# anthonyhu/tumblr-emotions

Measured on AMD Instinct MI355X. Metric: training samples/sec (224x224 img + 32-tok text, batch 256), higher is better.
Workload: dtype f32; 1 GPU; joint train step (fwd+bwd+all-reduce+Adam): Inception-v1 224x224x3 + 300-d embedding + LSTM-512, T=32, V=10000, 15 classes, batch 256 per GPU, reference freeze (<=Mixed_5b conv weights frozen, all BN betas trainable), dropout 0.8, BN train mode; global_batch=256, per_gpu_batch=256, parallelism=dp1, launch=eager

## Files before the change

### include/ds_kernels.h

```cpp
#ifndef DS_KERNELS_H
#define DS_KERNELS_H

#include <stddef.h>
#include <stdint.h>

#ifdef __cplusplus
extern "C" {
#endif

#define DS_OK 0
#define DS_ERR_ARG (-1)
#define DS_ERR_LAUNCH (-2)
#define DS_ERR_WORKSPACE (-3)

#define DS_DTYPE_F32 0
#define DS_DTYPE_BF16 1

#define DS_EPI_BIAS 1
#define DS_EPI_RELU 2
#define DS_EPI_ACCUM 4
#define DS_EPI_STATS 8
#define DS_EPI_MASK 16
#define DS_EPI_BNSUMS 32

int ds_version(void);
const char *ds_last_error(void);

typedef struct ds_conv_desc {
    int32_t N, H, W;
    int32_t Cin;
    int32_t ldx;
    int32_t KH, KW, stride;
    int32_t pad_t, pad_l;
    int32_t OH, OW;
    int32_t Cout;
    int32_t ldz;
    int64_t w_tap_stride;
    int32_t w_n_stride;
    int32_t w_k_stride;
    int32_t flip;
    int32_t fold_cin;
    int32_t flags;
    int32_t ldmask;
    int32_t splits;
    int64_t z_split_stride;
    int32_t tile_nt;
    int32_t grid_x;
    int32_t dtype;
    int32_t x_dtype;
    int32_t partials;
    const float *norm_rstd;
    const float *norm_shift;
    const float *mask_rstd;
    const float *mask_shift;
    const struct ds_bn_bwd_on_load *bnb;
    int32_t mask_dtype;
    int32_t z_dtype;
    uint8_t *pool_argmax;
    const struct ds_bn_finalize_in_launch *fin;
} ds_conv_desc;

typedef struct ds_bn_finalize_in_launch {
    const float *beta;
    float *mean, *rstd, *shift;
    float *moving_mean, *moving_var;
    uint32_t *ticket;
    int64_t count;
    float eps, decay;
} ds_bn_finalize_in_launch;

typedef struct ds_bn_bwd_on_load {
    const float *mean, *rstd, *shift;
    const float *coef;
    int32_t nseg;
    int32_t c_end[3];
    int32_t ld[3];
    const float *dy[3];
} ds_bn_bwd_on_load;

#ifdef DS_TUNING
int ds_debug_conv_set_tile(int mt, int nt);
int ds_debug_conv_set_path(int path);
int ds_debug_conv_set_wide(int mode);
int ds_debug_conv_wino_allow_ablation(int on);
int ds_debug_conv_wino4_set_nb(int nb);
int ds_debug_conv_bf16_set_max_nb(int nb);
#endif
int ds_conv_igemm_partials(const ds_conv_desc *d);
int ds_conv_igemm_bnsums_supported(const ds_conv_desc *d);
int ds_conv_igemm_norm_supported(const ds_conv_desc *d);
int ds_conv_igemm_bnb_supported(const ds_conv_desc *d);
int ds_conv_igemm_pool3_supported(const ds_conv_desc *d);
int ds_conv_igemm_finalize_tickets(const ds_conv_desc *d);
int ds_conv_igemm(const ds_conv_desc *d, const float *x, const float *w, float *z, const float *bias,
                  const float *mask, float *stats, const float *pivot, void *stream);

size_t ds_weights_bf16_bytes(int32_t Cin, int32_t Cout, int32_t taps, int32_t dgrad);
int ds_weights_to_bf16(const float *w, void *wb, int32_t Cin, int32_t Cout, int32_t taps, int32_t dgrad, void *stream);
int ds_conv_bf16_supported(const ds_conv_desc *d);
int ds_conv_bf16_partials(const ds_conv_desc *d);
int ds_conv_bf16(const ds_conv_desc *d, const void *x, const void *wb, float *z, const void *mask, float *stats,
                 const float *pivot, void *stream);

size_t ds_weights_f32x3_bytes(int32_t Cin, int32_t Cout, int32_t taps, int32_t dgrad);
int ds_weights_to_f32x3(const float *w, void *wb, int32_t Cin, int32_t Cout, int32_t taps, int32_t dgrad, void *stream);
int ds_conv_f32x3_supported(const ds_conv_desc *d);
int ds_conv_f32x3_partials(const ds_conv_desc *d);
int ds_conv_f32x3(const ds_conv_desc *d, const float *x, const void *wb, float *z, const float *mask, float *stats,
                  const float *pivot, void *stream);

#define DS_FP8_E4M3 0
#define DS_FP8_E5M2 1
#define DS_AMAX_FLOATS 512
int ds_absmax(const void *x, int64_t n, int32_t x_dtype, float *amax, void *stream);
size_t ds_weights_fp8_bytes(int32_t Cin, int32_t Cout, int32_t taps, int32_t dgrad);
int ds_weights_to_fp8(const float *w, void *wq, float *wscale, int32_t Cin, int32_t Cout, int32_t taps, int32_t dgrad,
                      void *stream);
int ds_conv_fp8_supported(const ds_conv_desc *d);
int ds_conv_fp8_partials(const ds_conv_desc *d);
int ds_conv_fp8(const ds_conv_desc *d, const void *x, const float *x_amax, int32_t a_format, const void *wq,
                const float *wscale, float *z, const void *mask, float *stats, const float *pivot, void *stream);

int ds_conv_stem_partials(int32_t N, int32_t OH, int32_t OW);
int ds_conv_stem(const float *x, const float *w, float *z, float *stats, const float *pivot, int32_t N, int32_t H,
                 int32_t W, int32_t cin_store, int32_t Cout, int32_t ldz, void *stream);
int ds_conv_stem_pool_supported(int32_t H, int32_t W);
int ds_conv_stem_pool_partials(int32_t N, int32_t OH, int32_t OW);
int ds_conv_stem_pool(const float *x, const float *w, float *zmax, float *stats, const float *pivot, int32_t N, int32_t H,
                      int32_t W, int32_t cin_store, int32_t Cout, int32_t ldz, void *stream);
int ds_conv_stem_pool_bf16(const float *x, const float *w, float *zmax, float *stats, const float *pivot, int32_t N, int32_t H,
                           int32_t W, int32_t cin_store, int32_t Cout, int32_t ldz, void *stream);
int ds_conv_stem_dgrad_supported(int32_t H, int32_t W);
int ds_conv_stem_dgrad(const float *dz, const float *w, float *dx, int32_t N, int32_t H, int32_t W, int32_t cin_store,
                       int32_t ldx, void *stream);
int ds_conv_stem_bf16_partials(int32_t N, int32_t OH, int32_t OW);
int ds_conv_stem_bf16(const float *x, const float *w, float *z, float *stats, const float *pivot, int32_t N, int32_t H, int32_t W,
                      int32_t cin_store, int32_t Cout, int32_t ldz, void *stream);

int ds_wino_transform_weights(const float *w, float *u, int32_t Cin, int32_t Cout, int32_t dgrad, void *stream);
int ds_conv_wino_partials(int32_t N, int32_t H, int32_t W);
int ds_conv_wino(const float *x, const float *u, float *z, float *stats, const float *pivot, const float *ymask,
                 int32_t N, int32_t H, int32_t W, int32_t Cin, int32_t ldx, int32_t Cout, int32_t ldz, int32_t flags,
                 void *stream);

int ds_conv_wino4_supported(int32_t H, int32_t W, int32_t Cin, int32_t Cout);
int ds_conv_wino4_prefer(int32_t N, int32_t H, int32_t W, int32_t Cin, int32_t Cout);
int ds_wino4_transform_weights(const float *w, float *u, int32_t Cin, int32_t Cout, int32_t dgrad, void *stream);
int ds_conv_wino4_partials(int32_t N, int32_t H, int32_t W);
int ds_conv_wino4(const float *x, const float *u, float *z, float *stats, const float *pivot, const float *ymask,
                  int32_t N, int32_t H, int32_t W, int32_t Cin, int32_t ldx, int32_t Cout, int32_t ldz, int32_t flags,
                  void *stream);
int ds_conv_wino4_splitk_choose(int32_t N, int32_t H, int32_t W, int32_t Cin, int32_t Cout);
int ds_conv_wino4_splitk_partials(int32_t N, int32_t H, int32_t W);
size_t ds_conv_wino4_splitk_workspace(int32_t N, int32_t H, int32_t W, int32_t Cout, int32_t splits);
int ds_conv_wino4_splitk(const float *x, const float *u, float *z, float *stats, const float *pivot, const float *ymask,
                         int32_t y_dtype, int32_t N, int32_t H, int32_t W, int32_t Cin, int32_t ldx, int32_t Cout, int32_t ldz,
                         int32_t flags, int32_t splits, void *ws, size_t ws_bytes, void *stream);
int ds_wino4_transform_weights_bf16x2(const float *w, void *u2, int32_t Cin, int32_t Cout, int32_t dgrad, void *stream);
int ds_conv_wino4_bf16x2(const float *x, const void *u2, float *z, float *stats, const float *pivot, const void *ymask,
                         int32_t y_dtype , int32_t N,
                         int32_t H, int32_t W, int32_t Cin, int32_t ldx, int32_t Cout, int32_t ldz, int32_t flags, void *stream);
int ds_conv_wino4_bf16x2_x16(const void *x16, const void *u2, float *z, float *stats, const float *pivot, const void *ymask,
                             int32_t y_dtype, int32_t N, int32_t H, int32_t W, int32_t Cin, int32_t ldx, int32_t Cout, int32_t ldz,
                             int32_t flags, void *stream);

#define DS_CONV_FWD 0
#define DS_CONV_DGRAD 1
#define DS_ARITH_F32 0
#define DS_ARITH_BF16 1
#define DS_ARITH_FP8 2
#define DS_ARITH_F32X3 3
#define DS_FAM_IGEMM 0
#define DS_FAM_WINO2 1
#define DS_FAM_WINO4 2
#define DS_FAM_STEM 3
#define DS_FAM_BF16D 4
#define DS_FAM_FP8D 5
#define DS_FAM_F32X3 6
#define DS_FAM_WINO4H 7
#define DS_FAM_STEM_POOL 8
#define DS_FAM_STEM_DGRAD 9
#define DS_PLAN_NO_WINO 1u
#define DS_PLAN_NO_WINO4 2u
#define DS_PLAN_NO_STEM_DIRECT 4u
#define DS_PLAN_NO_BF16_DIRECT 8u
#define DS_PLAN_ACT16 16u
#define DS_PLAN_FP8_EVERYWHERE 64u
#define DS_PLAN_FP8_WIDE_RULE 128u
#define DS_PLAN_NO_WINO4H 256u
#define DS_PLAN_STEM_POOL 512u
#define DS_PLAN_NO_SPLITK 1024u
#define DS_PLAN_PACKED_RGB 32u
typedef struct ds_conv_layer_plan {
    ds_conv_desc d;
    int32_t family;
    int32_t role, arith;
    int32_t partials;
    int32_t w_cin, w_cout, k;
    int32_t a_format;
    int32_t x16_ok;
    int64_t w_bytes;
    int64_t wscale_floats;
    double alg_flops;
    int32_t splitk;
    int32_t reserved0;
    int64_t ws_bytes;
} ds_conv_layer_plan;
typedef struct ds_conv_io {
    const float *bias;
    const float *mask;
    float *stats;
    const float *pivot;
    const float *x_amax;
    const float *wscale;
    const ds_bn_finalize_in_launch *fin;
    void *ws;
    size_t ws_bytes;
} ds_conv_io;
int ds_conv_plan(ds_conv_layer_plan *plan, int32_t role, int32_t arith, uint32_t options, int32_t N, int32_t H, int32_t W,
                 int32_t w_cin, int32_t w_cout, int32_t k, int32_t stride, int32_t ldx, int32_t ldz, int32_t flags);
int ds_conv_plan_set_flags(ds_conv_layer_plan *plan, int32_t flags);
int ds_conv_plan_enable_bnsums(ds_conv_layer_plan *plan, int32_t ldy);
int ds_conv_plan_norm_supported(const ds_conv_layer_plan *plan);
int ds_conv_plan_bnb_supported(const ds_conv_layer_plan *plan);
int ds_conv_plan_enable_pool3(ds_conv_layer_plan *plan, uint8_t *argmax);
int ds_conv_plan_finalize_tickets(const ds_conv_layer_plan *plan);
int ds_conv_prepare_weights(const ds_conv_layer_plan *plan, const float *w_hwio, void *w_prepared, float *wscale,
                            void *stream);
int ds_conv_run(const ds_conv_layer_plan *plan, const void *x, const void *w, float *z, const ds_conv_io *io, void *stream);

size_t ds_conv_wgrad_workspace(const ds_conv_desc *d);
int ds_conv_wgrad(const ds_conv_desc *d, const float *x, const float *dz, int32_t lddz, float *dw,
                  void *ws, size_t ws_bytes, void *stream);

int ds_bn_finalize(const float *stats, int32_t P, int64_t count, int32_t C, const float *beta, const float *pivot,
                   float eps, float decay, float *mean, float *rstd, float *shift, float *moving_mean,
                   float *moving_var, void *stream);

int ds_bn_finalize_centered(const float *stats, int32_t P, int64_t count, int32_t C, const float *beta, const float *pivot,
                            float eps, float decay, float *mean, float *rstd, float *shift, float *moving_mean,
                            float *moving_var, float *mean_c, float *shift_c, void *stream);
typedef struct ds_bn_finalize_job {
    const float *stats;
    int32_t P, C;
    int64_t count;
    const float *beta;
    const float *pivot;
    float *mean, *rstd, *shift;
    float *moving_mean, *moving_var;
} ds_bn_finalize_job;
int ds_bn_finalize_multi(const ds_bn_finalize_job *jobs, int32_t njobs, float eps, float decay, void *stream);

int ds_bn_finalize_apply_relu(const float *stats, int32_t P, int64_t count, int32_t C, const float *beta, const float *pivot,
                              float eps, float decay, float *mean, float *rstd, float *shift, float *moving_mean,
                              float *moving_var, const float *z, int64_t M, const struct ds_segments *dst, uint32_t *ticket,
                              void *stream);

typedef struct ds_segments {
    int32_t nseg;
    int32_t c_begin[4];
    int32_t c_end[4];
    int32_t ld[4];
    void *ptr[4];
    int32_t dtype[4];
    float *amax[4];
    const float *ptr2[4];
} ds_segments;
int ds_bn_apply_relu(const float *z, int64_t M, int32_t C, const float *rstd, const float *shift,
                     const ds_segments *dst, void *stream);
int ds_bn_apply_relu_z16(const void *z16, int64_t M, int32_t C, const float *rstd, const float *shift,
                         const ds_segments *dst, void *stream);
int ds_bn_infer_prepare(const float *beta, const float *moving_mean, const float *moving_var, float eps,
                        int32_t C, float *rstd, float *shift, void *stream);

int ds_bn_bwd_partials(int64_t M, int32_t C);
int ds_bn_bwd_reduce(const void *z, int32_t ldz, int32_t z_dtype, const ds_segments *dy, int64_t M, int32_t C,
                     const float *mean, const float *rstd, const float *shift, float *partials, void *stream);
int ds_bn_bwd_finalize(const float *partials, int32_t P, int64_t M, int32_t C, float *dbeta, float *coef,
                       void *stream);
typedef struct ds_bn_sum_segments {
    int32_t nseg;
    int32_t c_begin[4], c_end[4];
    int32_t P[4];
    int32_t kind[4];
    const float *s[4];
    const float *q[4];
    int32_t P2[4];
    const float *s2[4];
    const float *q2[4];
} ds_bn_sum_segments;
int ds_bn_bwd_finalize_segs(const ds_bn_sum_segments *sg, int64_t M, int32_t C, const float *beta, float *dbeta,
                            float *coef, void *stream);
int ds_bn_bwd_finalize_multi(const ds_bn_sum_segments *sg, int64_t M, int32_t C, const float *const *beta,
                             float *const *dbeta, float *coef, void *stream);
int ds_bn_bwd_finalize_apply(const ds_bn_sum_segments *sg, const float *beta, float *dbeta, const float *const *beta_v,
                             float *const *dbeta_v, float *coef, const float *z, int32_t ldz, const ds_segments *dy, int64_t M,
                             int32_t C, const float *mean, const float *rstd, const float *shift, void *dz, int32_t dz_dtype,
                             int32_t lddz, float *amax, uint32_t *ticket, void *stream);
int ds_bn_bwd_apply(const float *z, int32_t ldz, const ds_segments *dy, int64_t M, int32_t C, const float *mean,
                    const float *rstd, const float *shift, const float *coef, float *dz, float *amax, void *stream);
int ds_bn_bwd_apply_bf16(const float *z, int32_t ldz, const ds_segments *dy, int64_t M, int32_t C, const float *mean,
                         const float *rstd, const float *shift, const float *coef, void *dz16, int32_t lddz, float *amax,
                         void *stream);

int ds_bn_bwd_apply_z16(const void *z16, int32_t ldz, const ds_segments *dy, int64_t M, int32_t C, const float *mean,
                        const float *rstd, const float *shift, const float *coef, void *dz16, int32_t lddz, float *amax,
                        void *stream);

int ds_maxpool_fwd(const void *x, void *y, uint8_t *argmax, int32_t N, int32_t H, int32_t W, int32_t C,
                   int32_t k, int32_t stride, int32_t pad_t, int32_t pad_l, int32_t OH, int32_t OW,
                   int32_t act_dtype, void *stream);
int ds_maxpool_bn_relu_fwd(const float *z, const float *rstd, const float *shift, void *y, uint8_t *argmax,
                           int32_t N, int32_t H, int32_t W, int32_t C, int32_t k, int32_t stride, int32_t pad_t,
                           int32_t pad_l, int32_t OH, int32_t OW, int32_t y_dtype, float *amax, void *stream);
int ds_bn_pool_bwd_partials(int32_t N, int32_t OH, int32_t OW, int32_t C);
int ds_bn_pool_bwd_reduce(const float *z, const float *dpool, const uint8_t *argmax, int32_t N, int32_t H, int32_t W,
                          int32_t C, int32_t pad_t, int32_t pad_l, int32_t OH, int32_t OW, const float *mean,
                          const float *rstd, const float *shift, float *partials, void *stream);
int ds_bn_pool_bwd_apply(const float *z, const float *dpool, const uint8_t *argmax, int32_t N, int32_t H, int32_t W,
                         int32_t C, int32_t pad_t, int32_t pad_l, int32_t OH, int32_t OW, const float *mean,
                         const float *rstd, const float *shift, const float *coef, float *dz, void *stream);
int ds_maxpool_bwd(const float *dy, const uint8_t *argmax, float *dx, int32_t accumulate, int32_t N,
                   int32_t H, int32_t W, int32_t C, int32_t k, int32_t stride, int32_t pad_t, int32_t pad_l,
                   int32_t OH, int32_t OW, void *stream);

int ds_maxpool3_bwd_sums_partials(int32_t N, int32_t W, int32_t C);
int ds_maxpool3_bwd_sums(const float *dy, const uint8_t *argmax, float *dx, int32_t accumulate, const void *y,
                         int32_t y_dtype, int32_t N, int32_t H, int32_t W, int32_t C, float *partials, void *stream);

int ds_maxpool3_bwd_dy16(const void *dy16, const uint8_t *argmax, float *dx, int32_t accumulate, const void *y, int32_t y_dtype,
                         int32_t N, int32_t H, int32_t W, int32_t C, float *partials, void *stream);

int ds_avgpool_dropout_fwd(const float *x, int32_t N, int32_t HW, int32_t C, float keep, uint64_t seed,
                           const uint64_t *seed_dev, const float *mask_in, float *mask_out, float *out,
                           void *stream);
int ds_avgpool_dropout_bwd(const float *dout, const float *mask, int32_t N, int32_t HW, int32_t C,
                           float keep, float *dx, void *stream);

int ds_gather_rows(const float *table, const int64_t *ids, float *out, int32_t B, int32_t T, int32_t D,
                   int64_t table_rows, int32_t time_major, void *stream);

int ds_embedding_grad(const float *dx, const int64_t *ids, float *dtable, int32_t B, int32_t T, int32_t D,
                      int64_t table_rows, int32_t time_major, void *stream);

int ds_lstm_cell_fwd(float *gates, const float *rec_slabs, int32_t nslabs, int64_t slab_stride,
                     const float *c_prev, const float *h_prev, const int64_t *seq_len, int32_t t, int32_t B,
                     int32_t H, float forget_bias, float *c_out, float *h_out, void *stream);
int ds_lstm_cell_bwd(const float *acts, const float *c_t, const float *c_prev, const float *dh,
                     const float *dh_slabs, int32_t nslabs, int64_t slab_stride, const float *dc,
                     const int64_t *seq_len, int32_t t, int32_t B, int32_t H, float *dgates, float *dc_prev,
                     float *dh_carry, void *stream);

int ds_seq_sort_desc(const int64_t *seq_len, int32_t B, int32_t T, int32_t *perm, int64_t *len_sorted, void *stream);
int ds_permute_rows(const void *src, int64_t lds, void *dst, int64_t ldd, const int32_t *perm, int32_t rows, int32_t cols,
                    int32_t elem_bytes, int32_t gather, void *stream);
#define DS_LSTM_SKIP_MASKED 256
int ds_lstm_seq_supported(int32_t B, int32_t H);
size_t ds_lstm_seq_workspace(int32_t B, int32_t H);
int ds_lstm_seq_fwd(float *gates, const float *wh, int32_t ldw, float *h, float *c, const int64_t *seq_len, int32_t T,
                    int32_t B, int32_t H, float forget_bias, int32_t rows, void *ws, size_t ws_bytes, void *stream);
int ds_lstm_seq_bwd(const float *acts, const float *wh, int32_t ldw, const float *c, const float *dh_last,
                    int32_t ld_dh, const int64_t *seq_len, int32_t T, int32_t B, int32_t H, float *dgates, int32_t rows,
                    void *ws, size_t ws_bytes, void *stream);
int ds_lstm_seq_status(void *ws, int32_t B);
#ifdef DS_TUNING
int ds_debug_lstm_seq_set_profile(void *buf);
int ds_debug_lstm_seq_set_profile_bwd(void *buf);
#endif

int ds_softmax_ce(const float *logits, const int64_t *labels, int32_t B, int32_t C, float grad_scale,
                  const float *grad_scale_dev, float *loss, float *dlogits, void *stream);

int ds_adam_tf(float *theta, const float *g, float *m, float *v, int64_t n, int64_t n_wd, float wd,
               float grad_scale, float lr_t, const float *lr_t_dev, float beta1, float beta2, float eps,
               void *stream);

int ds_sumsq(const float *x, int64_t n, float *scratch, float *out, void *stream);
int ds_colsum(const float *x, int64_t M, int32_t C, int32_t ld, float *scratch, float *out, void *stream);
int ds_slab_epilogue(const float *slabs, int32_t splits, int64_t slab_stride, int32_t lds, int64_t M, int32_t N, float *out,
                     int32_t ldo, const float *bias, const float *mask, int32_t ldmask, int32_t flags, void *stream);
int ds_copy2d(const float *src, int32_t lds, float *dst, int32_t ldd, int64_t rows, int32_t cols,
              void *stream);
int ds_pad_channels(const float *src, int32_t cs, float *dst, int32_t cd, int64_t pixels, void *stream);
int ds_fill(float *dst, int64_t n, float value, void *stream);

#ifdef __cplusplus
}
#endif
#endif
```

### tumblr_emotions_amd/_lib.py

```python
import ctypes as C
import os

_HERE = os.path.dirname(os.path.abspath(__file__))
LIB_PATH = os.environ.get("DS_LIB") or os.path.join(_HERE, "libds_kernels.so")

def tuning_env(name, default=None):
    return os.environ.get(name, default) if os.environ.get("DS_LIB") else default


DS_EPI_BIAS, DS_EPI_RELU, DS_EPI_ACCUM, DS_EPI_STATS, DS_EPI_MASK, DS_EPI_BNSUMS = 1, 2, 4, 8, 16, 32
DS_DTYPE_F32, DS_DTYPE_BF16 = 0, 1
DS_FP8_E4M3, DS_FP8_E5M2 = 0, 1
DS_CONV_FWD, DS_CONV_DGRAD = 0, 1
DS_LSTM_SKIP_MASKED = 256
DS_ARITH_F32, DS_ARITH_BF16, DS_ARITH_FP8, DS_ARITH_F32X3 = 0, 1, 2, 3
DS_FAM_IGEMM, DS_FAM_WINO2, DS_FAM_WINO4, DS_FAM_STEM, DS_FAM_BF16D, DS_FAM_FP8D, DS_FAM_F32X3, DS_FAM_WINO4H, DS_FAM_STEM_POOL = range(9)
DS_FAM_STEM_DGRAD = 9
DS_PLAN_NO_WINO, DS_PLAN_NO_WINO4, DS_PLAN_NO_STEM_DIRECT, DS_PLAN_NO_BF16_DIRECT, DS_PLAN_ACT16, DS_PLAN_PACKED_RGB = 1, 2, 4, 8, 16, 32
DS_PLAN_FP8_EVERYWHERE, DS_PLAN_FP8_WIDE_RULE, DS_PLAN_NO_WINO4H, DS_PLAN_STEM_POOL = 64, 128, 256, 512
DS_PLAN_NO_SPLITK = 1024


class ConvDesc(C.Structure):
    _fields_ = [
        ("N", C.c_int32), ("H", C.c_int32), ("W", C.c_int32), ("Cin", C.c_int32), ("ldx", C.c_int32),
        ("KH", C.c_int32), ("KW", C.c_int32), ("stride", C.c_int32), ("pad_t", C.c_int32), ("pad_l", C.c_int32),
        ("OH", C.c_int32), ("OW", C.c_int32), ("Cout", C.c_int32), ("ldz", C.c_int32),
        ("w_tap_stride", C.c_int64), ("w_n_stride", C.c_int32), ("w_k_stride", C.c_int32),
        ("flip", C.c_int32), ("fold_cin", C.c_int32), ("flags", C.c_int32), ("ldmask", C.c_int32),
        ("splits", C.c_int32), ("z_split_stride", C.c_int64),
        ("tile_nt", C.c_int32), ("grid_x", C.c_int32), ("dtype", C.c_int32), ("x_dtype", C.c_int32),
        ("partials", C.c_int32),
        ("norm_rstd", C.c_void_p), ("norm_shift", C.c_void_p), ("mask_rstd", C.c_void_p), ("mask_shift", C.c_void_p),
        ("bnb", C.c_void_p), ("mask_dtype", C.c_int32), ("z_dtype", C.c_int32), ("pool_argmax", C.c_void_p), ("fin", C.c_void_p),
    ]


class BnBwdOnLoad(C.Structure):
    _fields_ = [("mean", C.c_void_p), ("rstd", C.c_void_p), ("shift", C.c_void_p), ("coef", C.c_void_p),
                ("nseg", C.c_int32), ("c_end", C.c_int32 * 3), ("ld", C.c_int32 * 3), ("dy", C.c_void_p * 3)]


class BnFinalizeInLaunch(C.Structure):
    _fields_ = [("beta", C.c_void_p), ("mean", C.c_void_p), ("rstd", C.c_void_p), ("shift", C.c_void_p),
                ("moving_mean", C.c_void_p), ("moving_var", C.c_void_p), ("ticket", C.c_void_p), ("count", C.c_int64),
                ("eps", C.c_float), ("decay", C.c_float)]


class LayerPlanStruct(C.Structure):
    _fields_ = [("d", ConvDesc), ("family", C.c_int32), ("role", C.c_int32), ("arith", C.c_int32), ("partials", C.c_int32),
                ("w_cin", C.c_int32), ("w_cout", C.c_int32), ("k", C.c_int32), ("a_format", C.c_int32), ("x16_ok", C.c_int32),
                ("w_bytes", C.c_int64), ("wscale_floats", C.c_int64), ("alg_flops", C.c_double), ("splitk", C.c_int32),
                ("reserved0", C.c_int32), ("ws_bytes", C.c_int64)]


class ConvIO(C.Structure):
    _fields_ = [("bias", C.c_void_p), ("mask", C.c_void_p), ("stats", C.c_void_p), ("pivot", C.c_void_p),
                ("x_amax", C.c_void_p), ("wscale", C.c_void_p), ("fin", C.c_void_p), ("ws", C.c_void_p), ("ws_bytes", C.c_size_t)]


class Segments(C.Structure):
    _fields_ = [("nseg", C.c_int32), ("c_begin", C.c_int32 * 4), ("c_end", C.c_int32 * 4),
                ("ld", C.c_int32 * 4), ("ptr", C.c_void_p * 4), ("dtype", C.c_int32 * 4),
                ("amax", C.c_void_p * 4), ("ptr2", C.c_void_p * 4)]


class BnFinalizeJob(C.Structure):
    _fields_ = [("stats", C.c_void_p), ("P", C.c_int32), ("C", C.c_int32), ("count", C.c_int64), ("beta", C.c_void_p),
                ("pivot", C.c_void_p), ("mean", C.c_void_p), ("rstd", C.c_void_p), ("shift", C.c_void_p),
                ("moving_mean", C.c_void_p), ("moving_var", C.c_void_p)]


class SumSegments(C.Structure):
    _fields_ = [("nseg", C.c_int32), ("c_begin", C.c_int32 * 4), ("c_end", C.c_int32 * 4), ("P", C.c_int32 * 4),
                ("kind", C.c_int32 * 4), ("s", C.c_void_p * 4), ("q", C.c_void_p * 4), ("P2", C.c_int32 * 4),
                ("s2", C.c_void_p * 4), ("q2", C.c_void_p * 4)]


_P = C.c_void_p
_i32, _i64, _f32, _u64 = C.c_int32, C.c_int64, C.c_float, C.c_uint64
_CD = C.POINTER(ConvDesc)
_SG = C.POINTER(Segments)
_SS = C.POINTER(SumSegments)
_LP = C.POINTER(LayerPlanStruct)
_IO = C.POINTER(ConvIO)

SIGNATURES = {
    "ds_version": (C.c_int, []),
    "ds_last_error": (C.c_char_p, []),
    "ds_conv_igemm_partials": (C.c_int, [_CD]),
    "ds_conv_igemm_bnsums_supported": (C.c_int, [_CD]),
    "ds_conv_igemm_norm_supported": (C.c_int, [_CD]),
    "ds_conv_igemm_bnb_supported": (C.c_int, [_CD]),
    "ds_conv_igemm_pool3_supported": (C.c_int, [_CD]),
    "ds_conv_igemm_finalize_tickets": (C.c_int, [_CD]),
    "ds_conv_igemm": (C.c_int, [_CD, _P, _P, _P, _P, _P, _P, _P, _P]),
    "ds_weights_bf16_bytes": (C.c_size_t, [_i32, _i32, _i32, _i32]),
    "ds_weights_to_bf16": (C.c_int, [_P, _P, _i32, _i32, _i32, _i32, _P]),
    "ds_conv_bf16_supported": (C.c_int, [_CD]),
    "ds_conv_bf16_partials": (C.c_int, [_CD]),
    "ds_conv_bf16": (C.c_int, [_CD, _P, _P, _P, _P, _P, _P, _P]),
    "ds_weights_f32x3_bytes": (C.c_size_t, [_i32, _i32, _i32, _i32]),
    "ds_weights_to_f32x3": (C.c_int, [_P, _P, _i32, _i32, _i32, _i32, _P]),
    "ds_conv_f32x3_supported": (C.c_int, [_CD]),
    "ds_conv_f32x3_partials": (C.c_int, [_CD]),
    "ds_conv_f32x3": (C.c_int, [_CD, _P, _P, _P, _P, _P, _P, _P]),
    "ds_absmax": (C.c_int, [_P, _i64, _i32, _P, _P]),
    "ds_weights_fp8_bytes": (C.c_size_t, [_i32, _i32, _i32, _i32]),
    "ds_weights_to_fp8": (C.c_int, [_P, _P, _P, _i32, _i32, _i32, _i32, _P]),
    "ds_conv_fp8_supported": (C.c_int, [_CD]),
    "ds_conv_fp8_partials": (C.c_int, [_CD]),
    "ds_conv_fp8": (C.c_int, [_CD, _P, _P, _i32, _P, _P, _P, _P, _P, _P, _P]),
    "ds_conv_stem_partials": (C.c_int, [_i32, _i32, _i32]),
    "ds_conv_stem_bf16_partials": (C.c_int, [_i32, _i32, _i32]),
    "ds_conv_stem": (C.c_int, [_P, _P, _P, _P, _P, _i32, _i32, _i32, _i32, _i32, _i32, _P]),
    "ds_conv_stem_bf16": (C.c_int, [_P, _P, _P, _P, _P, _i32, _i32, _i32, _i32, _i32, _i32, _P]),
    "ds_conv_stem_pool_supported": (C.c_int, [_i32, _i32]),
    "ds_conv_stem_pool_partials": (C.c_int, [_i32, _i32, _i32]),
    "ds_conv_stem_pool": (C.c_int, [_P, _P, _P, _P, _P, _i32, _i32, _i32, _i32, _i32, _i32, _P]),
    "ds_conv_stem_pool_bf16": (C.c_int, [_P, _P, _P, _P, _P, _i32, _i32, _i32, _i32, _i32, _i32, _P]),
    "ds_conv_stem_dgrad_supported": (C.c_int, [_i32, _i32]),
    "ds_conv_stem_dgrad": (C.c_int, [_P, _P, _P, _i32, _i32, _i32, _i32, _i32, _P]),
    "ds_wino_transform_weights": (C.c_int, [_P, _P, _i32, _i32, _i32, _P]),
    "ds_conv_wino_partials": (C.c_int, [_i32, _i32, _i32]),
    "ds_conv_wino": (C.c_int, [_P, _P, _P, _P, _P, _P, _i32, _i32, _i32, _i32, _i32, _i32, _i32, _i32, _P]),
    "ds_conv_wino4_supported": (C.c_int, [_i32, _i32, _i32, _i32]),
    "ds_conv_wino4_prefer": (C.c_int, [_i32, _i32, _i32, _i32, _i32]),
    "ds_wino4_transform_weights": (C.c_int, [_P, _P, _i32, _i32, _i32, _P]),
    "ds_conv_wino4_partials": (C.c_int, [_i32, _i32, _i32]),
    "ds_conv_wino4_splitk_choose": (C.c_int, [_i32, _i32, _i32, _i32, _i32]),
    "ds_conv_wino4_splitk_partials": (C.c_int, [_i32, _i32, _i32]),
    "ds_conv_wino4_splitk_workspace": (C.c_size_t, [_i32, _i32, _i32, _i32, _i32]),
    "ds_conv_wino4_splitk": (C.c_int, [_P, _P, _P, _P, _P, _P, _i32, _i32, _i32, _i32, _i32, _i32, _i32, _i32, _i32, _i32, _P, C.c_size_t, _P]),
    "ds_conv_wino4": (C.c_int, [_P, _P, _P, _P, _P, _P, _i32, _i32, _i32, _i32, _i32, _i32, _i32, _i32, _P]),
    "ds_conv_wino4_bf16x2": (C.c_int, [_P, _P, _P, _P, _P, _P, _i32, _i32, _i32, _i32, _i32, _i32, _i32, _i32, _i32, _P]),
    "ds_conv_wino4_bf16x2_x16": (C.c_int, [_P, _P, _P, _P, _P, _P, _i32, _i32, _i32, _i32, _i32, _i32, _i32, _i32, _i32, _P]),
    "ds_wino4_transform_weights_bf16x2": (C.c_int, [_P, _P, _i32, _i32, _i32, _P]),
    "ds_conv_plan": (C.c_int, [_LP, _i32, _i32, C.c_uint32] + [_i32] * 10),
    "ds_conv_plan_set_flags": (C.c_int, [_LP, _i32]),
    "ds_conv_plan_enable_bnsums": (C.c_int, [_LP, _i32]),
    "ds_conv_plan_norm_supported": (C.c_int, [_LP]),
    "ds_conv_plan_bnb_supported": (C.c_int, [_LP]),
    "ds_conv_plan_enable_pool3": (C.c_int, [_LP, C.c_void_p]),
    "ds_conv_plan_finalize_tickets": (C.c_int, [_LP]),
    "ds_conv_prepare_weights": (C.c_int, [_LP, _P, _P, _P, _P]),
    "ds_conv_run": (C.c_int, [_LP, _P, _P, _P, _IO, _P]),
    "ds_conv_wgrad_workspace": (C.c_size_t, [_CD]),
    "ds_conv_wgrad": (C.c_int, [_CD, _P, _P, _i32, _P, _P, C.c_size_t, _P]),
    "ds_bn_finalize": (C.c_int, [_P, _i32, _i64, _i32, _P, _P, _f32, _f32, _P, _P, _P, _P, _P, _P]),
    "ds_bn_finalize_centered": (C.c_int, [_P, _i32, _i64, _i32, _P, _P, _f32, _f32, _P, _P, _P, _P, _P, _P, _P, _P]),
    "ds_bn_apply_relu": (C.c_int, [_P, _i64, _i32, _P, _P, _SG, _P]),
    "ds_bn_apply_relu_z16": (C.c_int, [_P, _i64, _i32, _P, _P, _SG, _P]),
    "ds_bn_bwd_apply_z16": (C.c_int, [_P, _i32, _SG, _i64, _i32, _P, _P, _P, _P, _P, _i32, _P, _P]),
    "ds_bn_infer_prepare": (C.c_int, [_P, _P, _P, _f32, _i32, _P, _P, _P]),
    "ds_bn_bwd_partials": (C.c_int, [_i64, _i32]),
    "ds_bn_bwd_reduce": (C.c_int, [_P, _i32, _i32, _SG, _i64, _i32, _P, _P, _P, _P, _P]),
    "ds_bn_bwd_finalize_segs": (C.c_int, [_SS, _i64, _i32, _P, _P, _P, _P]),
    "ds_bn_bwd_finalize": (C.c_int, [_P, _i32, _i64, _i32, _P, _P, _P]),
    "ds_bn_bwd_finalize_multi": (C.c_int, [_SS, _i64, _i32, _P, _P, _P, _P]),
    "ds_bn_finalize_multi": (C.c_int, [_P, _i32, _f32, _f32, _P]),
    "ds_bn_finalize_apply_relu": (C.c_int, [_P, _i32, _i64, _i32, _P, _P, _f32, _f32, _P, _P, _P, _P, _P, _P, _i64, _SG, _P, _P]),
    "ds_bn_bwd_finalize_apply": (C.c_int, [_SS, _P, _P, _P, _P, _P, _P, _i32, _SG, _i64, _i32, _P, _P, _P, _P, _i32, _i32, _P, _P, _P]),
    "ds_bn_bwd_apply": (C.c_int, [_P, _i32, _SG, _i64, _i32, _P, _P, _P, _P, _P, _P, _P]),
    "ds_bn_bwd_apply_bf16": (C.c_int, [_P, _i32, _SG, _i64, _i32, _P, _P, _P, _P, _P, _i32, _P, _P]),
    "ds_maxpool_fwd": (C.c_int, [_P, _P, _P] + [_i32] * 11 + [_P]),
    "ds_maxpool_bn_relu_fwd": (C.c_int, [_P, _P, _P, _P, _P] + [_i32] * 11 + [_P, _P]),
    "ds_bn_pool_bwd_partials": (C.c_int, [_i32, _i32, _i32, _i32]),
    "ds_bn_pool_bwd_reduce": (C.c_int, [_P, _P, _P] + [_i32] * 8 + [_P, _P, _P, _P, _P]),
    "ds_bn_pool_bwd_apply": (C.c_int, [_P, _P, _P] + [_i32] * 8 + [_P, _P, _P, _P, _P, _P]),
    "ds_maxpool_bwd": (C.c_int, [_P, _P, _P] + [_i32] * 11 + [_P]),
    "ds_maxpool3_bwd_sums_partials": (C.c_int, [_i32, _i32, _i32]),
    "ds_maxpool3_bwd_sums": (C.c_int, [_P, _P, _P, _i32, _P, _i32, _i32, _i32, _i32, _i32, _P, _P]),
    "ds_maxpool3_bwd_dy16": (C.c_int, [_P, _P, _P, _i32, _P, _i32, _i32, _i32, _i32, _i32, _P, _P]),
    "ds_avgpool_dropout_fwd": (C.c_int, [_P, _i32, _i32, _i32, _f32, _u64, _P, _P, _P, _P, _P]),
    "ds_avgpool_dropout_bwd": (C.c_int, [_P, _P, _i32, _i32, _i32, _f32, _P, _P]),
    "ds_gather_rows": (C.c_int, [_P, _P, _P, _i32, _i32, _i32, _i64, _i32, _P]),
    "ds_embedding_grad": (C.c_int, [_P, _P, _P, _i32, _i32, _i32, _i64, _i32, _P]),
    "ds_lstm_cell_fwd": (C.c_int, [_P, _P, _i32, _i64, _P, _P, _P, _i32, _i32, _i32, _f32, _P, _P, _P]),
    "ds_lstm_cell_bwd": (C.c_int, [_P, _P, _P, _P, _P, _i32, _i64, _P, _P, _i32, _i32, _i32, _P, _P, _P, _P]),
    "ds_seq_sort_desc": (C.c_int, [_P, _i32, _i32, _P, _P, _P]),
    "ds_permute_rows": (C.c_int, [_P, _i64, _P, _i64, _P, _i32, _i32, _i32, _i32, _P]),
    "ds_lstm_seq_supported": (C.c_int, [_i32, _i32]),
    "ds_lstm_seq_workspace": (C.c_size_t, [_i32, _i32]),
    "ds_lstm_seq_fwd": (C.c_int, [_P, _P, _i32, _P, _P, _P, _i32, _i32, _i32, _f32, _i32, _P, C.c_size_t, _P]),
    "ds_lstm_seq_bwd": (C.c_int, [_P, _P, _i32, _P, _P, _i32, _P, _i32, _i32, _i32, _P, _i32, _P, C.c_size_t, _P]),
    "ds_lstm_seq_status": (C.c_int, [_P, _i32]),
    "ds_softmax_ce": (C.c_int, [_P, _P, _i32, _i32, _f32, _P, _P, _P, _P]),
    "ds_adam_tf": (C.c_int, [_P, _P, _P, _P, _i64, _i64, _f32, _f32, _f32, _P, _f32, _f32, _f32, _P]),
    "ds_sumsq": (C.c_int, [_P, _i64, _P, _P, _P]),
    "ds_colsum": (C.c_int, [_P, _i64, _i32, _i32, _P, _P, _P]),
    "ds_slab_epilogue": (C.c_int, [_P, _i32, _i64, _i32, _i64, _i32, _P, _i32, _P, _P, _i32, _i32, _P]),
    "ds_copy2d": (C.c_int, [_P, _i32, _P, _i32, _i64, _i32, _P]),
    "ds_pad_channels": (C.c_int, [_P, _i32, _P, _i32, _i64, _P]),
    "ds_fill": (C.c_int, [_P, _i64, _f32, _P]),
}

_lib = None


DEBUG_SIGNATURES = {
    "ds_debug_conv_set_tile": (C.c_int, [C.c_int, C.c_int]),
    "ds_debug_conv_set_path": (C.c_int, [C.c_int]),
    "ds_debug_conv_set_wide": (C.c_int, [C.c_int]),
    "ds_debug_conv_wino_allow_ablation": (C.c_int, [C.c_int]),
    "ds_debug_conv_wino4_set_nb": (C.c_int, [C.c_int]),
    "ds_debug_conv_bf16_set_max_nb": (C.c_int, [C.c_int]),
    "ds_debug_lstm_seq_set_profile": (C.c_int, [_P]),
    "ds_debug_lstm_seq_set_profile_bwd": (C.c_int, [_P]),
}
TUNING_LIB_PATH = os.path.join(_HERE, "libds_kernels_tuning.so")
_tuning = None


def _bind(lib, table):
    for name, (res, args) in table.items():
        fn = getattr(lib, name)
        fn.restype = res
        fn.argtypes = args


def load_tuning():
    global _tuning
    if _tuning is None:
        if not os.path.exists(TUNING_LIB_PATH):
            raise RuntimeError("tumblr_emotions_amd: %s not found -- `make -C tumblr_emotions_amd/csrc` builds it" % TUNING_LIB_PATH)
        lib = C.CDLL(TUNING_LIB_PATH)
        _bind(lib, SIGNATURES)
        _bind(lib, DEBUG_SIGNATURES)
        _tuning = lib
    return _tuning


class tuning_library:

    def __enter__(self):
        global _lib
        self._saved = load()
        _lib = load_tuning()
        return _lib

    def __exit__(self, *exc):
        global _lib
        _lib = self._saved
        return False


def load():
    global _lib
    if _lib is not None:
        return _lib
    if not os.path.exists(LIB_PATH):
        raise RuntimeError(
            "tumblr_emotions_amd: %s not found -- build it with `python -c 'import __graft_entry__ as g; "
            "g.build()'` or `make -C tumblr_emotions_amd/csrc`.  There is no CPU fallback." % LIB_PATH)
    if os.environ.get("DS_LIB"):
        import sys
        sys.stderr.write("tumblr_emotions_amd: DS_LIB overrides the kernel library: %s\n" % LIB_PATH)
    lib = C.CDLL(LIB_PATH)
    _bind(lib, SIGNATURES)
    if hasattr(lib, "ds_debug_conv_set_tile"):
        _bind(lib, DEBUG_SIGNATURES)
    _lib = lib
    return lib


def check(rc, what):
    if rc != 0:
        raise RuntimeError("%s failed (%d): %s" % (what, rc, load().ds_last_error().decode()))
```

### tumblr_emotions_amd/csrc/conv_wgrad.hip

```cpp
#include <stdio.h>
#include <stdlib.h>
#include "ds_common.h"

typedef float f32x16 __attribute__((ext_vector_type(16)));
typedef float f32x4 __attribute__((ext_vector_type(4)));
typedef unsigned int u32x4 __attribute__((ext_vector_type(4)));

namespace {

constexpr int TJ = 128;
constexpr int TP = 16;

struct WgradParams {
    ds_conv_desc d;
    const float *x;
    const float *dz;
    float *out;
    int lddz;
    int M;
    int ci_tiles;
    int pix_per_split;
    int x_vec, z_vec;
    unsigned x_bytes, z_bytes;
    float inv_ohw, inv_ow;
    int slabs;
};

constexpr unsigned kOOB = 0x80000000u;

__device__ __forceinline__ __amdgpu_buffer_rsrc_t make_srd(const void *p, unsigned bytes) {
    return __builtin_amdgcn_make_buffer_rsrc(const_cast<void *>(p), 0, (int)bytes, 0x00020000);
}

__device__ __forceinline__ f32x4 load4(__amdgpu_buffer_rsrc_t r, unsigned off, bool ok, bool vec, int valid) {
    if (vec) return __builtin_bit_cast(f32x4, __builtin_amdgcn_raw_buffer_load_b128(r, ok ? off : kOOB, 0, 0));
    f32x4 v;
#pragma unroll
    for (int j = 0; j < 4; ++j)
        v[j] = __builtin_bit_cast(float, __builtin_amdgcn_raw_buffer_load_b32(r, (ok && j < valid) ? off + 4 * j : kOOB, 0, 0));
    return v;
}

__device__ __forceinline__ int fdiv(int a, int b, float inv) {
    int q = (int)((float)a * inv);
    int r = a - q * b;
    if (r < 0) --q;
    if (r >= b) ++q;
    return q;
}

template <int TIT>
__global__ __launch_bounds__(256) void conv_wgrad_kernel(const WgradParams p) {
    constexpr int LDX = TIT + 4, LDZ = TJ + 4;
    constexpr int WNW = TIT == 128 ? 2 : 4;
    constexpr int CW = TJ / WNW;
    constexpr int BS = CW / 32;
    constexpr int XQ = TIT / 4;
    constexpr int XROWS = 256 / XQ;
    constexpr int XP = TP / XROWS;
    __shared__ __attribute__((aligned(16))) float smem[2 * TP * LDX + 2 * TP * LDZ];
    float *Xs = smem;
    float *Zs = smem + 2 * TP * LDX;
    const ds_conv_desc &d = p.d;
    const int tid = threadIdx.x, lane = tid & 63;
    const int wave = __builtin_amdgcn_readfirstlane(tid >> 6);
    const int wm = TIT == 128 ? wave >> 1 : 0, wn = TIT == 128 ? wave & 1 : wave;
    const int li = lane & 31, lk = lane >> 5;
    const int tap = blockIdx.x / p.ci_tiles;
    const int i0 = (blockIdx.x % p.ci_tiles) * TIT;
    const int j0 = blockIdx.y * TJ;
    const int split = blockIdx.z;
    const int dh = tap / d.KW, dw = tap % d.KW;
    const int ohw = d.OH * d.OW;
    const int m_begin = split * p.pix_per_split;
    int m_end = m_begin + p.pix_per_split;
    if (m_end > p.M) m_end = p.M;

    int it_valid = (d.Cin - (i0 + wm * 64) + 31) / 32;
    it_valid = it_valid < 0 ? 0 : (it_valid > 2 ? 2 : it_valid);
    int jt_valid = (d.Cout - (j0 + wn * CW) + 31) / 32;
    jt_valid = jt_valid < 0 ? 0 : (jt_valid > BS ? BS : jt_valid);

    f32x16 acc[2][BS];
#pragma unroll
    for (int a = 0; a < 2; ++a)
#pragma unroll
        for (int b = 0; b < BS; ++b)
#pragma unroll
            for (int r = 0; r < 16; ++r) acc[a][b][r] = 0.f;

    const int xrow = tid / XQ, xc4 = (tid % XQ) * 4;
    const int zrow = tid >> 5, zc4 = (tid & 31) * 4;
    f32x4 rx[XP], rz[2];
    const __amdgpu_buffer_rsrc_t srd_x = make_srd(p.x, p.x_bytes);
    const __amdgpu_buffer_rsrc_t srd_z = make_srd(p.dz, p.z_bytes);
    const int cx = i0 + xc4, cz = j0 + zc4;
    const bool small = p.M < (1 << 24);

    auto load_tile = [&](int mt0) {
#pragma unroll
        for (int i = 0; i < XP; ++i) {
            const int m = mt0 + xrow + XROWS * i;
            const bool rv = m < m_end;
            const int mm = rv ? m : 0;
            const int n = small ? fdiv(mm, ohw, p.inv_ohw) : mm / ohw;
            const int r = mm - n * ohw;
            const int oh = small ? fdiv(r, d.OW, p.inv_ow) : r / d.OW;
            const int ow = r - oh * d.OW;
            const int ih = oh * d.stride - d.pad_t + dh, iw = ow * d.stride - d.pad_l + dw;
            const int iwc = d.fold_cin > 0 ? iw + cx / d.fold_cin : iw;
            const bool okx = rv && (unsigned)ih < (unsigned)d.H && (unsigned)iwc < (unsigned)d.W && cx < d.Cin;
            const unsigned offx = (unsigned)(((n * d.H + ih) * d.W + iw) * d.ldx + cx);
            rx[i] = load4(srd_x, offx * 4u, okx, p.x_vec, d.Cin - cx);
        }
#pragma unroll
        for (int i = 0; i < 2; ++i) {
            const int m = mt0 + zrow + 8 * i;
            const bool okz = m < m_end && cz < d.Cout;
            const unsigned offz = (unsigned)(m < m_end ? m : 0) * (unsigned)p.lddz + (unsigned)cz;
            rz[i] = load4(srd_z, offz * 4u, okz, p.z_vec, d.Cout - cz);
        }
    };
    auto store_tile = [&](int buf) {
#pragma unroll
        for (int i = 0; i < XP; ++i)
            *reinterpret_cast<f32x4 *>(Xs + (buf * TP + xrow + XROWS * i) * LDX + xc4) = rx[i];
#pragma unroll
        for (int i = 0; i < 2; ++i)
            *reinterpret_cast<f32x4 *>(Zs + (buf * TP + zrow + 8 * i) * LDZ + zc4) = rz[i];
    };
    auto compute = [&](int buf) {
        const float *xs = Xs + buf * TP * LDX + wm * 64 + li;
        const float *zs = Zs + buf * TP * LDZ + wn * CW + li;
#pragma unroll
        for (int s = 0; s < TP / 2; ++s) {
            const int row = 2 * s + lk;
            float af[2], bf[BS];
            af[0] = xs[row * LDX];
            af[1] = xs[row * LDX + 32];
#pragma unroll
            for (int b = 0; b < BS; ++b) bf[b] = zs[row * LDZ + 32 * b];
#pragma unroll
            for (int a = 0; a < 2; ++a)
#pragma unroll
                for (int b = 0; b < BS; ++b)
                    if (a < it_valid && b < jt_valid)
                        acc[a][b] = __builtin_amdgcn_mfma_f32_32x32x2f32(af[a], bf[b], acc[a][b], 0, 0, 0);
        }
    };

    const int KT = (m_end - m_begin + TP - 1) / TP;
    if (KT > 0) {
        load_tile(m_begin);
        store_tile(0);
        __syncthreads();
        for (int kt = 0; kt < KT; ++kt) {
            const int cur = kt & 1;
            if (kt + 1 < KT) load_tile(m_begin + (kt + 1) * TP);
            compute(cur);
            if (kt + 1 < KT) store_tile(cur ^ 1);
            __syncthreads();
        }
    }

    float *out = p.out + (int64_t)split * (d.KH * d.KW) * d.Cin * d.Cout + (int64_t)tap * d.Cin * d.Cout;
#pragma unroll
    for (int a = 0; a < 2; ++a)
#pragma unroll
        for (int b = 0; b < BS; ++b) {
            const int col = j0 + wn * CW + b * 32 + li;
#pragma unroll
            for (int r = 0; r < 16; ++r) {
                const int row = i0 + wm * 64 + a * 32 + (r & 3) + 8 * (r >> 2) + 4 * lk;
                if (row < d.Cin && col < d.Cout) out[(int64_t)row * d.Cout + col] = acc[a][b][r];
            }
        }
}


#ifndef DS_WG_U
#define DS_WG_U 4
#endif
template <int W>
__device__ __forceinline__ f32x4 loadw(__amdgpu_buffer_rsrc_t r, unsigned off) {
    f32x4 v = {0.f, 0.f, 0.f, 0.f};
    if constexpr (W == 4) {
        v = __builtin_bit_cast(f32x4, __builtin_amdgcn_raw_buffer_load_b128(r, off, 0, 0));
    } else if constexpr (W == 2) {
        typedef unsigned int u32x2 __attribute__((ext_vector_type(2)));
        typedef float f32x2 __attribute__((ext_vector_type(2)));
        const f32x2 t = __builtin_bit_cast(f32x2, __builtin_amdgcn_raw_buffer_load_b64(r, off, 0, 0));
        v[0] = t[0]; v[1] = t[1];
    } else {
        v[0] = __builtin_bit_cast(float, __builtin_amdgcn_raw_buffer_load_b32(r, off, 0, 0));
    }
    return v;
}

template <int AI, int BJ>
__global__ __launch_bounds__(256, (AI * BJ > 8) ? 1 : 2) void wgrad_direct_kernel(const WgradParams p) {
    constexpr int NACC = AI * BJ, U = DS_WG_U;
    __shared__ __attribute__((aligned(16))) float red[2 * NACC * 16 * 64];
    const ds_conv_desc &d = p.d;
    const int tid = threadIdx.x, lane = tid & 63;
    const int wave = __builtin_amdgcn_readfirstlane(tid >> 6);
    const int li = lane & 31, lk = lane >> 5;
    const int co_tiles = (d.Cout + 32 * BJ - 1) / (32 * BJ);
    const int split = (int)(blockIdx.x % (unsigned)p.slabs);
    int bid = (int)(blockIdx.x / (unsigned)p.slabs);
    const int jt = bid % co_tiles; bid /= co_tiles;
    const int itile = bid % p.ci_tiles;
    const int tap = bid / p.ci_tiles;
    const int dh = tap / d.KW, dw = tap % d.KW;
    const int ci0 = itile * 32 * AI, co0 = jt * 32 * BJ;
    const int ci = ci0 + AI * li, co = co0 + BJ * li;
    const bool ci_ok = ci < d.Cin, co_ok = co < d.Cout;
    const __amdgpu_buffer_rsrc_t srd_x = make_srd(p.x, p.x_bytes);
    const __amdgpu_buffer_rsrc_t srd_z = make_srd(p.dz, p.z_bytes);

    const int m_begin = split * p.pix_per_split;
    int m_end = m_begin + p.pix_per_split;
    if (m_end > p.M) m_end = p.M;
    int q = (m_end - m_begin + 3) / 4;
    q = (q + 1) & ~1;
    const int wb = m_begin + wave * q;
    int we = wb + q;
    if (we > m_end) we = m_end;
    const int steps = we > wb ? (we - wb + 1) / 2 : 0;

    int m = wb + lk;
    const int ohw = d.OH * d.OW;
    int oh = 0, ow = 0;
    unsigned offx, offz;
    {
        const int mm = m < p.M ? m : 0;
        const int n = mm / ohw;
        const int r = mm - n * ohw;
        oh = r / d.OW;
        ow = r - oh * d.OW;
        const int ih = oh * d.stride - d.pad_t + dh, iw = ow * d.stride - d.pad_l + dw;
        offx = ((unsigned)((n * d.H + ih) * d.W + iw) * (unsigned)d.ldx + (unsigned)ci) * 4u;
        offz = ((unsigned)mm * (unsigned)p.lddz + (unsigned)co) * 4u;
    }
    const unsigned ldx4 = (unsigned)d.ldx * 4u;
    const unsigned step_x = 2u * (unsigned)d.stride * ldx4;
    const unsigned row_x = (unsigned)((d.W - d.OW) * d.stride) * ldx4;
    const unsigned img_x = (unsigned)((d.H - d.OH * d.stride) * d.W) * ldx4;
    const unsigned step_z = 2u * (unsigned)p.lddz * 4u;
    auto lo_of = [](int pad, int tap, int stride) { const int v = pad - tap; return v <= 0 ? 0 : (v + stride - 1) / stride; };
    auto hi_of = [](int pad, int tap, int stride, int ext, int oext) {
        const int v = ext - 1 + pad - tap;
        const int h = v < 0 ? -1 : v / stride;
        return h > oext - 1 ? oext - 1 : h;
    };
    const int lo_h = lo_of(d.pad_t, dh, d.stride), lo_w = lo_of(d.pad_l, dw, d.stride);
    const unsigned span_h = (unsigned)(hi_of(d.pad_t, dh, d.stride, d.H, d.OH) - lo_h);
    const unsigned span_w = (unsigned)(hi_of(d.pad_l, dw, d.stride, d.W, d.OW) - lo_w);
    const int OWc = d.OW, OHc = d.OH;
    auto offsets = [&](unsigned &ox, unsigned &oz) {
        const bool mv = m < we;
        const bool in = (unsigned)(oh - lo_h) <= span_h && (unsigned)(ow - lo_w) <= span_w;
        oz = (mv && co_ok) ? offz : kOOB;
        ox = (mv && ci_ok && in) ? offx : kOOB;
        m += 2;
        offz += step_z;
        offx += step_x;
        ow += 2;
#pragma unroll
        for (int rep = 0; rep < 2; ++rep) {
            if (rep == 1 && OWc > 1) break;
            const bool wrap = ow >= OWc;
            ow = wrap ? ow - OWc : ow;
            oh += wrap ? 1 : 0;
            offx += wrap ? row_x : 0u;
            const bool wrap2 = oh >= OHc;
            oh = wrap2 ? oh - OHc : oh;
            offx += wrap2 ? img_x : 0u;
        }
    };

    f32x16 acc[AI][BJ];
#pragma unroll
    for (int a = 0; a < AI; ++a)
#pragma unroll
        for (int b = 0; b < BJ; ++b)
#pragma unroll
            for (int r = 0; r < 16; ++r) acc[a][b][r] = 0.f;

    f32x4 xa[U], zb[U];
#pragma unroll
    for (int u = 0; u < U; ++u) {
        unsigned ox, oz;
        offsets(ox, oz);
        xa[u] = loadw<AI>(srd_x, ox);
        zb[u] = loadw<BJ>(srd_z, oz);
    }
    for (int s = 0; s < steps; s += U) {
#pragma unroll
        for (int u = 0; u < U; ++u) {
            const f32x4 a4 = xa[u], b4 = zb[u];
            unsigned ox, oz;
            offsets(ox, oz);
            xa[u] = loadw<AI>(srd_x, ox);
            zb[u] = loadw<BJ>(srd_z, oz);
#pragma unroll
            for (int a = 0; a < AI; ++a)
#pragma unroll
                for (int b = 0; b < BJ; ++b)
                    acc[a][b] = __builtin_amdgcn_mfma_f32_32x32x2f32(a4[a], b4[b], acc[a][b], 0, 0, 0);
        }
    }

    auto put = [&](int slot) {
#pragma unroll
        for (int a = 0; a < AI; ++a)
#pragma unroll
            for (int b = 0; b < BJ; ++b)
#pragma unroll
                for (int r4 = 0; r4 < 4; ++r4) {
                    f32x4 v = {acc[a][b][4 * r4], acc[a][b][4 * r4 + 1], acc[a][b][4 * r4 + 2], acc[a][b][4 * r4 + 3]};
                    *reinterpret_cast<f32x4 *>(red + ((slot * NACC + a * BJ + b) * 4 + r4) * 256 + lane * 4) = v;
                }
    };
    auto get = [&](int slot) {
#pragma unroll
        for (int a = 0; a < AI; ++a)
#pragma unroll
            for (int b = 0; b < BJ; ++b)
#pragma unroll
                for (int r4 = 0; r4 < 4; ++r4) {
                    const f32x4 v = *reinterpret_cast<const f32x4 *>(red + ((slot * NACC + a * BJ + b) * 4 + r4) * 256 + lane * 4);
#pragma unroll
                    for (int e = 0; e < 4; ++e) acc[a][b][4 * r4 + e] += v[e];
                }
    };
    if (wave >= 2) put(wave - 2);
    __syncthreads();
    if (wave < 2) get(wave);
    __syncthreads();
    if (wave == 1) put(0);
    __syncthreads();
    if (wave != 0) return;
    get(0);

    float *out = p.out + (int64_t)split * (d.KH * d.KW) * d.Cin * d.Cout + (int64_t)tap * d.Cin * d.Cout;
    if (!co_ok) return;
#pragma unroll
    for (int a = 0; a < AI; ++a)
#pragma unroll
        for (int r = 0; r < 16; ++r) {
            const int row = ci0 + AI * ((r & 3) + 8 * (r >> 2) + 4 * lk) + a;
            if (row < d.Cin) {
                float *o = out + (int64_t)row * d.Cout + co;
                if constexpr (BJ == 4) {
                    *reinterpret_cast<f32x4 *>(o) = f32x4{acc[a][0][r], acc[a][1][r], acc[a][2][r], acc[a][3][r]};
                } else if constexpr (BJ == 2) {
                    typedef float f32x2 __attribute__((ext_vector_type(2)));
                    *reinterpret_cast<f32x2 *>(o) = f32x2{acc[a][0][r], acc[a][1][r]};
                } else {
                    *o = acc[a][0][r];
                }
            }
        }
}

__global__ __launch_bounds__(256) void splitk_reduce_kernel(const float *ws, float *dw, int64_t n, int splits) {
    for (int64_t i = (int64_t)blockIdx.x * 256 + threadIdx.x; i < n; i += (int64_t)gridDim.x * 256) {
        float s = 0.f;
        for (int k = 0; k < splits; ++k) s += ws[(int64_t)k * n + i];
        dw[i] = s;
    }
}

int pick_ti(const ds_conv_desc *d) {
    const int p128 = (d->Cin + 127) / 128 * 128, p64 = (d->Cin + 63) / 64 * 64;
    return (p128 - p64) * 5 >= p128 ? 64 : 128;
}

int pick_splits(const ds_conv_desc *d, int64_t M) {
    const int ti = pick_ti(d);
    const int tiles = d->KH * d->KW * ((d->Cin + ti - 1) / ti) * ((d->Cout + TJ - 1) / TJ);
    static int occ = 0, minpix = 0;
    if (!occ) {
        const char *e = ds::tune_env("DS_WGRAD_OCC");
        occ = e ? atoi(e) : 3;
        e = ds::tune_env("DS_WGRAD_MINPIX");
        minpix = e ? atoi(e) : 64;
    }
    int splits = (occ * ds::kCUs + tiles - 1) / tiles;
    const int max_splits = (int)((M + minpix - 1) / minpix);
    if (splits > max_splits) splits = max_splits;
    if (splits < 1) splits = 1;
    return splits;
}

struct WgradPlan {
    int direct;
    int ai, bj;
    int splits;
};

int max_width(int C, int ld, uintptr_t ptr) {
    for (int w = 4; w > 1; w >>= 1)
        if (C % w == 0 && ld % w == 0 && (ptr & (4 * w - 1)) == 0) return w;
    return 1;
}

bool direct_ok(const ds_conv_desc *d, int64_t M) {
    static int mode = -1;
    if (mode < 0) {
        const char *e = ds::tune_env("DS_WGRAD_DIRECT");
        mode = e ? atoi(e) : 1;
    }
    return mode && d->fold_cin == 0 && M >= 512;
}

WgradPlan plan_direct(const ds_conv_desc *d, int64_t M, int wx, int wz, int only_ai = 0, int only_bj = 0) {
    WgradPlan best = {};
    double best_cost = 1e30;
    static const int kSlabs[] = {1, 2, 4, 8, 16, 24, 32, 40, 48, 56, 64};
    const double wbytes = (double)d->KH * d->KW * d->Cin * d->Cout * 4.0;
    for (int ai = 1; ai <= wx; ai *= 2)
        for (int bj = 1; bj <= wz; bj *= 2) {
            if ((only_ai && ai != only_ai) || (only_bj && bj != only_bj)) continue;
            const int nacc = ai * bj;
            const int occ = nacc > 8 ? 1 : (nacc > 4 ? 2 : 3);
            const int tiles = d->KH * d->KW * ((d->Cin + 32 * ai - 1) / (32 * ai)) * ((d->Cout + 32 * bj - 1) / (32 * bj));
            for (int slabs : kSlabs) {
                if (slabs > 1 && M / slabs < 256) break;
                const int xcds = slabs >= 8 ? 8 : slabs;
                const double per_xcd = (double)tiles * slabs / 8.0;
                const double slots = 32.0 * occ;
                double rounds = (double)(int64_t)(per_xcd / slots);
                if (rounds * slots < per_xcd) rounds += 1.0;
                const double steps = (double)M / slabs / 8.0;
                const double step_cycles = nacc * 64.0 > 160.0 ? nacc * 64.0 : 160.0;
                const double t_wg = steps * step_cycles + 1500.0 + nacc * 350.0;
                const double t_red = slabs > 1 ? 6000.0 + slabs * wbytes / 1500.0 : 0.0;
                const double cost = rounds * t_wg + t_red;
                (void)xcds;
                if (cost < best_cost) {
                    best_cost = cost;
                    best.direct = 1; best.ai = ai; best.bj = bj; best.splits = slabs;
                }
            }
        }
    return best;
}

WgradPlan plan_wgrad(const ds_conv_desc *d, int64_t M, const float *x, const float *dz, int lddz, const float *dw,
                     const void *ws) {
    if (direct_ok(d, M)) {
        const uintptr_t zalign = (uintptr_t)dz | (uintptr_t)dw | (uintptr_t)ws;
        const int wx = max_width(d->Cin, d->ldx, (uintptr_t)x), wz = max_width(d->Cout, lddz, zalign);
        WgradPlan pl = plan_direct(d, M, wx, wz);
        if (const char *e = ds::tune_env("DS_WGRAD_FORCE")) {
            int a = 0, b = 0, sl = 0;
            if (sscanf(e, "%d,%d,%d", &a, &b, &sl) == 3) {
                if ((a && a <= wx) || (b && b <= wz)) {
                    const WgradPlan f = plan_direct(d, M, wx, wz, a <= wx ? a : 0, b <= wz ? b : 0);
                    if (f.direct) pl = f;
                }
                if (sl) pl.splits = sl;
            }
        }
        return pl;
    }
    WgradPlan pl = {};
    pl.splits = pick_splits(d, M);
    return pl;
}

}

extern "C" size_t ds_conv_wgrad_workspace(const ds_conv_desc *d) {
    const int64_t M = (int64_t)d->N * d->OH * d->OW;
    int splits = pick_splits(d, M);
    if (direct_ok(d, M)) {
        splits = 1;
        for (int wx = 1; wx <= 4; wx *= 2)
            for (int wz = 1; wz <= 4; wz *= 2) {
                const int sp = plan_direct(d, M, wx, wz).splits;
                splits = sp > splits ? sp : splits;
            }
    }
    if (splits == 1) return 0;
    return (size_t)splits * d->KH * d->KW * d->Cin * d->Cout * sizeof(float);
}

extern "C" int ds_conv_wgrad(const ds_conv_desc *d, const float *x, const float *dz, int32_t lddz, float *dw,
                             void *ws, size_t ws_bytes, void *stream) {
    DS_REQUIRE(d && x && dz && dw, "ds_conv_wgrad: null argument");
    const int64_t M = (int64_t)d->N * d->OH * d->OW;
    DS_REQUIRE(M < (1ll << 31), "ds_conv_wgrad: M too large");
    DS_REQUIRE(d->fold_cin == 0 || (d->KW == 1 && d->ldx == d->fold_cin && d->fold_cin % 4 == 0 && d->Cin % d->fold_cin == 0),
               "ds_conv_wgrad: fold_cin needs KW=1, ldx==fold_cin, fold_cin %% 4 == 0");
    const WgradPlan pl = plan_wgrad(d, M, x, dz, lddz, dw, ws);
    if (ds::tune_env("DS_WGRAD_DEBUG"))
        fprintf(stderr, "wgrad M=%lld Cin=%d Cout=%d k=%d: direct=%d ai=%d bj=%d slabs=%d\n", (long long)M, d->Cin, d->Cout, d->KH,
                pl.direct, pl.ai, pl.bj, pl.splits);
    const int splits = pl.splits;
    const size_t need = splits == 1 ? 0 : (size_t)splits * d->KH * d->KW * d->Cin * d->Cout * sizeof(float);
    if (need > 0 && (ws == nullptr || ws_bytes < need)) {
        ds::set_error("ds_conv_wgrad: workspace %zu bytes < required %zu", ws_bytes, need);
        return DS_ERR_WORKSPACE;
    }
    WgradParams p;
    p.d = *d;
    p.x = x; p.dz = dz; p.lddz = lddz;
    p.out = splits == 1 ? dw : (float *)ws;
    p.M = (int)M;
    const int64_t x_elems = ((int64_t)d->N * d->H * d->W - 1) * d->ldx + d->Cin;
    const int64_t z_elems = (M - 1) * lddz + d->Cout;
    DS_REQUIRE(x_elems * 4 < (1ll << 31) && z_elems * 4 < (1ll << 31), "ds_conv_wgrad: operand larger than 2 GiB (split the batch)");
    p.x_bytes = (unsigned)(x_elems * 4);
    p.z_bytes = (unsigned)(z_elems * 4);
    p.inv_ohw = 1.0f / (float)(d->OH * d->OW);
    p.inv_ow = 1.0f / (float)d->OW;
    p.x_vec = (d->ldx % 4 == 0) && (d->Cin % 4 == 0) && (((uintptr_t)x & 15) == 0);
    p.z_vec = (lddz % 4 == 0) && (d->Cout % 4 == 0) && (((uintptr_t)dz & 15) == 0);
    hipStream_t s = (hipStream_t)stream;
    int pps = (int)((M + splits - 1) / splits);
    if (pl.direct) {
        p.ci_tiles = (d->Cin + 32 * pl.ai - 1) / (32 * pl.ai);
        p.pix_per_split = (pps + 7) / 8 * 8;
        const int co_tiles = (d->Cout + 32 * pl.bj - 1) / (32 * pl.bj);
        p.slabs = splits;
        const dim3 grid((unsigned)(d->KH * d->KW * p.ci_tiles * co_tiles * splits));
#define DS_WG(A, B) if (pl.ai == A && pl.bj == B) hipLaunchKernelGGL((wgrad_direct_kernel<A, B>), grid, dim3(256), 0, s, p);
        DS_WG(4, 4) DS_WG(4, 2) DS_WG(4, 1) DS_WG(2, 4) DS_WG(2, 2) DS_WG(2, 1) DS_WG(1, 4) DS_WG(1, 2) DS_WG(1, 1)
#undef DS_WG
    } else {
        const int ti = pick_ti(d);
        p.ci_tiles = (d->Cin + ti - 1) / ti;
        p.pix_per_split = ((pps + TP - 1) / TP) * TP;
        dim3 grid(d->KH * d->KW * p.ci_tiles, (d->Cout + TJ - 1) / TJ, splits);
        if (ti == 64) hipLaunchKernelGGL(conv_wgrad_kernel<64>, grid, dim3(256), 0, s, p);
        else hipLaunchKernelGGL(conv_wgrad_kernel<128>, grid, dim3(256), 0, s, p);
    }
    if (splits > 1) {
        const int64_t n = (int64_t)d->KH * d->KW * d->Cin * d->Cout;
        hipLaunchKernelGGL(splitk_reduce_kernel, dim3(ds::stream_grid(n, 256)), dim3(256), 0, s,
                           (const float *)ws, dw, n, splits);
    }
    return ds::check_launch("ds_conv_wgrad");
}
```

### tumblr_emotions_amd/csrc/text_misc.hip

```cpp
#include <stdlib.h>
#include "ds_common.h"

namespace {

template <int VEC, bool NT = true, bool OUTORDER = false>
__global__ __launch_bounds__(256) void gather_rows_kernel(const float *table, const int64_t *ids, float *out, int B,
                                                          int T, int D, int64_t rows, int time_major, int rpw) {
    typedef float vec_t __attribute__((ext_vector_type(VEC)));
    const int lane = threadIdx.x & 63;
    const int64_t wave = ((int64_t)blockIdx.x * 256 + threadIdx.x) >> 6;
    const int64_t total = (int64_t)B * T;
    int64_t r = wave * rpw;
    const int64_t r1 = r + rpw < total ? r + rpw : total;
    if (r >= r1) return;
    const int DV = D / VEC;
    int b, t;
    if (OUTORDER) { t = (int)(r / B); b = (int)(r - (int64_t)t * B); }
    else { b = (int)(r / T); t = (int)(r - (int64_t)b * T); }
    constexpr int U = 4;
    if (VEC == 4 && DV <= 128) {
        const float *srcA[U], *srcB[U];
        float *dstA[U], *dstB[U];
        bool okA[U], okB[U];
        vec_t a0[U], a1[U], b0[U], b1[U];
        auto fetch = [&](int64_t rr, const float *(&src)[U], float *(&dst)[U], bool (&ok)[U], vec_t (&v0)[U], vec_t (&v1)[U]) {
#pragma unroll
            for (int u = 0; u < U; ++u) {
                const bool in = rr + u < r1;
                const int64_t id = in ? ids[OUTORDER ? (int64_t)b * T + t : rr + u] : -1;
                ok[u] = id >= 0 && id < rows;
                src[u] = table + (ok[u] ? id : 0) * D;
                dst[u] = in ? out + (OUTORDER ? rr + u : (time_major ? (int64_t)t * B + b : rr + u)) * D : nullptr;
                if (OUTORDER) { if (++b == B) { b = 0; ++t; } }
                else if (++t == T) { t = 0; ++b; }
            }
#pragma unroll
            for (int u = 0; u < U; ++u) {
                v0[u] = vec_t(0.f);
                v1[u] = vec_t(0.f);
                if (lane < DV && ok[u]) v0[u] = *reinterpret_cast<const vec_t *>(src[u] + lane * VEC);
                if (64 + lane < DV && ok[u]) v1[u] = *reinterpret_cast<const vec_t *>(src[u] + (64 + lane) * VEC);
            }
        };
        auto put = [&](float *(&dst)[U], vec_t (&v0)[U], vec_t (&v1)[U]) {
#pragma unroll
            for (int u = 0; u < U; ++u) {
                if (!dst[u]) continue;
                if (lane < DV) {
                    if (NT) __builtin_nontemporal_store(v0[u], reinterpret_cast<vec_t *>(dst[u] + lane * VEC));
                    else *reinterpret_cast<vec_t *>(dst[u] + lane * VEC) = v0[u];
                }
                if (64 + lane < DV) {
                    if (NT) __builtin_nontemporal_store(v1[u], reinterpret_cast<vec_t *>(dst[u] + (64 + lane) * VEC));
                    else *reinterpret_cast<vec_t *>(dst[u] + (64 + lane) * VEC) = v1[u];
                }
            }
        };
        fetch(r, srcA, dstA, okA, a0, a1);
        for (; r < r1; r += 2 * U) {
            if (r + U < r1) fetch(r + U, srcB, dstB, okB, b0, b1);
            put(dstA, a0, a1);
            if (r + U >= r1) break;
            if (r + 2 * U < r1) fetch(r + 2 * U, srcA, dstA, okA, a0, a1);
            put(dstB, b0, b1);
        }
        return;
    }
    for (; r < r1; r += U) {
        const float *src[U];
        float *dst[U];
        bool ok[U];
#pragma unroll
        for (int u = 0; u < U; ++u) {
            const bool in = r + u < r1;
            const int64_t id = in ? ids[OUTORDER ? (int64_t)b * T + t : r + u] : -1;
            ok[u] = id >= 0 && id < rows;
            src[u] = table + (ok[u] ? id : 0) * D;
            dst[u] = in ? out + (OUTORDER ? r + u : (time_major ? (int64_t)t * B + b : r + u)) * D : nullptr;
            if (OUTORDER) { if (++b == B) { b = 0; ++t; } }
            else if (++t == T) { t = 0; ++b; }
        }
        for (int v0 = 0; v0 < DV; v0 += 64) {
            const int v = v0 + lane;
            vec_t val[U];
#pragma unroll
            for (int u = 0; u < U; ++u) {
                val[u] = vec_t(0.f);
                if (v < DV && ok[u]) val[u] = *reinterpret_cast<const vec_t *>(src[u] + v * VEC);
            }
#pragma unroll
            for (int u = 0; u < U; ++u)
                if (v < DV && dst[u]) {
                    if (NT) __builtin_nontemporal_store(val[u], reinterpret_cast<vec_t *>(dst[u] + v * VEC));
                    else *reinterpret_cast<vec_t *>(dst[u] + v * VEC) = val[u];
                }
        }
    }
}

template <int NQ>
__global__ __launch_bounds__(256) void embedding_grad_kernel(const float *dx, const int64_t *ids, float *dtable, int B,
                                                             int T, int D, int64_t rows, int time_major) {
    const int lane = threadIdx.x & 63;
    const int64_t v = (int64_t)blockIdx.x * 4 + (threadIdx.x >> 6);
    if (v >= rows) return;
    float acc[NQ];
#pragma unroll
    for (int q = 0; q < NQ; ++q) acc[q] = 0.f;
    const int BT = B * T;
    for (int base = 0; base < BT; base += 64) {
        const int pos = base + lane;
        const int64_t id = pos < BT ? ids[pos] : -1;
        unsigned long long mask = __ballot(id == v);
        while (mask) {
            const int j = __ffsll((long long)mask) - 1;
            mask &= mask - 1;
            const int p = base + j;
            const int b = p / T, t = p - b * T;
            const float *src = dx + (time_major ? (int64_t)t * B + b : (int64_t)p) * D;
#pragma unroll
            for (int q = 0; q < NQ; ++q) {
                const int c = lane + 64 * q;
                if (c < D) acc[q] += src[c];
            }
        }
    }
#pragma unroll
    for (int q = 0; q < NQ; ++q) {
        const int c = lane + 64 * q;
        if (c < D) dtable[v * D + c] = acc[q];
    }
}

__device__ __forceinline__ float sigmoidf_(float x) { return 1.f / (1.f + __expf(-x)); }

__global__ __launch_bounds__(256) void lstm_cell_fwd_kernel(float *gates, const float *rec, int nslabs,
                                                            int64_t slab_stride, const float *c_prev,
                                                            const float *h_prev, const int64_t *seq_len, int t, int B,
                                                            int H, float forget_bias, float *c_out, float *h_out) {
    const int64_t total = (int64_t)B * H;
    for (int64_t i = (int64_t)blockIdx.x * 256 + threadIdx.x; i < total; i += (int64_t)gridDim.x * 256) {
        const int b = (int)(i / H), h = (int)(i - (int64_t)b * H);
        float *g = gates + (int64_t)b * 4 * H + h;
        float pi = g[0], pj = g[H], pf = g[2 * H], po = g[3 * H];
        for (int s = 0; s < nslabs; ++s) {
            const float *r = rec + s * slab_stride + (int64_t)b * 4 * H + h;
            pi += r[0]; pj += r[H]; pf += r[2 * H]; po += r[3 * H];
        }
        const float si = sigmoidf_(pi);
        const float tj = tanhf(pj);
        const float sf = sigmoidf_(pf + forget_bias);
        const float so = sigmoidf_(po);
        const float cp = c_prev[i], hp = h_prev[i];
        const float cn = cp * sf + si * tj;
        const float hn = tanhf(cn) * so;
        const bool live = (int64_t)t < seq_len[b];
        g[0] = si;
        g[H] = tj;
        g[2 * H] = sf;
        g[3 * H] = so;
        c_out[i] = live ? cn : cp;
        h_out[i] = live ? hn : hp;
    }
}

__global__ __launch_bounds__(256) void lstm_cell_bwd_kernel(const float *acts, const float *c_t, const float *c_prev,
                                                            const float *dh, const float *dh_slabs, int nslabs,
                                                            int64_t slab_stride, const float *dc,
                                                            const int64_t *seq_len, int t, int B, int H,
                                                            float *dgates, float *dc_prev, float *dh_carry) {
    const int64_t total = (int64_t)B * H;
    for (int64_t i = (int64_t)blockIdx.x * 256 + threadIdx.x; i < total; i += (int64_t)gridDim.x * 256) {
        const int b = (int)(i / H), h = (int)(i - (int64_t)b * H);
        const float *a = acts + (int64_t)b * 4 * H + h;
        float *dg = dgates + (int64_t)b * 4 * H + h;
        const bool live = (int64_t)t < seq_len[b];
        float dhv = dh[i];
        for (int s = 0; s < nslabs; ++s) dhv += dh_slabs[s * slab_stride + i];
        const float dcv = dc[i];
        if (live) {
            const float si = a[0], tj = a[H], sf = a[2 * H], so = a[3 * H];
            const float tc = tanhf(c_t[i]);
            const float dct = dcv + dhv * so * (1.f - tc * tc);
            dg[0] = dct * tj * si * (1.f - si);
            dg[H] = dct * si * (1.f - tj * tj);
            dg[2 * H] = dct * c_prev[i] * sf * (1.f - sf);
            dg[3 * H] = dhv * tc * so * (1.f - so);
            dc_prev[i] = dct * sf;
            dh_carry[i] = 0.f;
        } else {
            dg[0] = 0.f;
            dg[H] = 0.f;
            dg[2 * H] = 0.f;
            dg[3 * H] = 0.f;
            dc_prev[i] = dcv;
            dh_carry[i] = dhv;
        }
    }
}

__global__ __launch_bounds__(256) void softmax_ce_kernel(const float *logits, const int64_t *labels, int B, int C,
                                                         float grad_scale, const float *grad_scale_dev,
                                                         float *loss, float *dlogits) {
    __shared__ float red[256];
    if (grad_scale_dev) grad_scale *= grad_scale_dev[0];
    float acc = 0.f;
    for (int b = threadIdx.x; b < B; b += 256) {
        const float *z = logits + (int64_t)b * C;
        float m = -INFINITY;
        for (int c = 0; c < C; ++c) m = fmaxf(m, z[c]);
        float s = 0.f;
        for (int c = 0; c < C; ++c) s += expf(z[c] - m);
        const int64_t yl = labels[b];
        const bool yok = yl >= 0 && yl < C;
        const int y = yok ? (int)yl : -1;
        acc += yok ? (m + logf(s)) - z[y] : NAN;
        if (dlogits) {
            const float k = grad_scale / (float)B, inv = 1.f / s;
            for (int c = 0; c < C; ++c)
                dlogits[(int64_t)b * C + c] = (expf(z[c] - m) * inv - (c == y ? 1.f : 0.f)) * k;
        }
    }
    red[threadIdx.x] = acc;
    __syncthreads();
    for (int o = 128; o > 0; o >>= 1) {
        if (threadIdx.x < o) red[threadIdx.x] += red[threadIdx.x + o];
        __syncthreads();
    }
    if (threadIdx.x == 0 && loss) loss[0] = red[0] / (float)B;
}

__global__ __launch_bounds__(256) void adam_tf_kernel(float *theta, const float *g, float *m, float *v, int64_t n,
                                                      int64_t n_wd, float wd, float grad_scale, float lr_t,
                                                      const float *lr_t_dev, float b1, float b2, float eps) {
    if (lr_t_dev) lr_t = lr_t_dev[0];
    for (int64_t i = (int64_t)blockIdx.x * 256 + threadIdx.x; i < n; i += (int64_t)gridDim.x * 256) {
        const float w = theta[i];
        float gi = g[i] * grad_scale;
        if (i < n_wd) gi += wd * w;
        const float mi = b1 * m[i] + (1.f - b1) * gi;
        const float vi = b2 * v[i] + (1.f - b2) * gi * gi;
        m[i] = mi;
        v[i] = vi;
        theta[i] = w - lr_t * mi / (sqrtf(vi) + eps);
    }
}

constexpr int kSumsqBlocks = 256;

__global__ __launch_bounds__(256) void sumsq_stage1(const float *x, int64_t n, float *partials) {
    __shared__ float red[256];
    float acc = 0.f;
    for (int64_t i = (int64_t)blockIdx.x * 256 + threadIdx.x; i < n; i += (int64_t)gridDim.x * 256) acc += x[i] * x[i];
    red[threadIdx.x] = acc;
    __syncthreads();
    for (int o = 128; o > 0; o >>= 1) {
        if (threadIdx.x < o) red[threadIdx.x] += red[threadIdx.x + o];
        __syncthreads();
    }
    if (threadIdx.x == 0) partials[blockIdx.x] = red[0];
}

__global__ __launch_bounds__(256) void sum_stage2(const float *partials, int n, float *out) {
    __shared__ double red[256];
    double acc = 0.0;
    for (int i = threadIdx.x; i < n; i += 256) acc += (double)partials[i];
    red[threadIdx.x] = acc;
    __syncthreads();
    for (int o = 128; o > 0; o >>= 1) {
        if (threadIdx.x < o) red[threadIdx.x] += red[threadIdx.x + o];
        __syncthreads();
    }
    if (threadIdx.x == 0) out[0] = (float)red[0];
}

__global__ __launch_bounds__(256) void colsum_stage1(const float *x, int64_t M, int C, int ld, int rows_per_split,
                                                     float *partials) {
    __shared__ float red[4][64];
    const int cl = threadIdx.x & 63, rl = threadIdx.x >> 6;
    const int c = blockIdx.x * 64 + cl;
    const int64_t r0 = (int64_t)blockIdx.y * rows_per_split;
    int64_t r1 = r0 + rows_per_split;
    if (r1 > M) r1 = M;
    float acc = 0.f;
    if (c < C)
        for (int64_t r = r0 + rl; r < r1; r += 4) acc += x[r * ld + c];
    red[rl][cl] = acc;
    __syncthreads();
    if (rl == 0 && c < C) partials[(int64_t)blockIdx.y * C + c] = red[0][cl] + red[1][cl] + red[2][cl] + red[3][cl];
}

__global__ __launch_bounds__(256) void colsum_small_kernel(const float *x, int64_t M, int C, int ld, int rows_per_split,
                                                           int RS, float *out) {
    __shared__ float red[4][64];
    const int cl = threadIdx.x & 63, rl = threadIdx.x >> 6;
    const int c = blockIdx.x * 64 + cl;
    double total = 0.0;
    for (int s = 0; s < RS; ++s) {
        const int64_t r0 = (int64_t)s * rows_per_split;
        int64_t r1 = r0 + rows_per_split;
        if (r1 > M) r1 = M;
        float acc = 0.f;
        if (c < C)
            for (int64_t r = r0 + rl; r < r1; r += 4) acc += x[r * ld + c];
        __syncthreads();
        red[rl][cl] = acc;
        __syncthreads();
        if (rl == 0) total += (double)(red[0][cl] + red[1][cl] + red[2][cl] + red[3][cl]);
    }
    if (rl == 0 && c < C) out[c] = (float)total;
}

__global__ __launch_bounds__(256) void colsum_stage2(const float *partials, int RS, int C, float *out) {
    const int c = blockIdx.x * 256 + threadIdx.x;
    if (c >= C) return;
    double acc = 0.0;
    for (int s = 0; s < RS; ++s) acc += (double)partials[(int64_t)s * C + c];
    out[c] = (float)acc;
}

__global__ __launch_bounds__(256) void copy2d_kernel(const float *src, int lds, float *dst, int ldd, int64_t rows,
                                                     int cols) {
    const int64_t total = rows * cols;
    for (int64_t i = (int64_t)blockIdx.x * 256 + threadIdx.x; i < total; i += (int64_t)gridDim.x * 256) {
        const int64_t r = i / cols;
        const int c = (int)(i - r * cols);
        dst[r * ldd + c] = src[r * lds + c];
    }
}

__global__ __launch_bounds__(256) void pad_channels_kernel(const float *src, int cs, float *dst, int cd,
                                                           int64_t pixels) {
    const int64_t total = pixels * cd;
    for (int64_t i = (int64_t)blockIdx.x * 256 + threadIdx.x; i < total; i += (int64_t)gridDim.x * 256) {
        const int64_t p = i / cd;
        const int c = (int)(i - p * cd);
        dst[i] = c < cs ? src[p * cs + c] : 0.f;
    }
}

__global__ __launch_bounds__(256) void fill_kernel(float *dst, int64_t n, float value) {
    for (int64_t i = (int64_t)blockIdx.x * 256 + threadIdx.x; i < n; i += (int64_t)gridDim.x * 256) dst[i] = value;
}

}

extern "C" int ds_gather_rows(const float *table, const int64_t *ids, float *out, int32_t B, int32_t T, int32_t D,
                              int64_t table_rows, int32_t time_major, void *stream) {
    DS_REQUIRE(table && ids && out && B > 0 && T > 0 && D > 0 && table_rows > 0, "ds_gather_rows: bad argument");
    hipStream_t s = (hipStream_t)stream;
    const bool a16 = (((uintptr_t)table | (uintptr_t)out) & 15) == 0, a8 = (((uintptr_t)table | (uintptr_t)out) & 7) == 0;
    const int64_t total = (int64_t)B * T;
    int rpw = (int)((total + (int64_t)ds::kCUs * 32 * 4 - 1) / ((int64_t)ds::kCUs * 32 * 4));
    rpw = rpw < 4 ? 4 : (rpw > 16 ? 16 : rpw);
    const int64_t waves = (total + rpw - 1) / rpw;
    const dim3 grid((unsigned)((waves + 3) / 4));
    static int plain = -1;
    if (plain < 0) {
        const char *e = ds::tune_env("DS_GATHER_PLAIN_STORES");
        plain = e ? atoi(e) : 0;
    }
    static int outorder = -1;
    if (outorder < 0) {
        const char *e = ds::tune_env("DS_GATHER_OUTORDER");
        outorder = e ? atoi(e) : 1;
    }
    if (D % 4 == 0 && a16 && !plain && time_major && outorder == 1) {
        hipLaunchKernelGGL((gather_rows_kernel<4, true, true>), grid, dim3(256), 0, s, table, ids, out, B, T, D, table_rows, time_major, rpw);
    } else if (D % 4 == 0 && a16 && time_major && outorder == 2) {
        hipLaunchKernelGGL((gather_rows_kernel<4, false, true>), grid, dim3(256), 0, s, table, ids, out, B, T, D, table_rows, time_major, rpw);
    } else if (D % 4 == 0 && a16 && plain) {
        hipLaunchKernelGGL((gather_rows_kernel<4, false>), grid, dim3(256), 0, s, table, ids, out, B, T, D, table_rows, time_major, rpw);
    } else if (D % 4 == 0 && a16) {
        hipLaunchKernelGGL(gather_rows_kernel<4>, grid, dim3(256), 0, s, table, ids, out, B, T, D, table_rows, time_major, rpw);
    } else if (D % 2 == 0 && a8) {
        hipLaunchKernelGGL(gather_rows_kernel<2>, grid, dim3(256), 0, s, table, ids, out, B, T, D, table_rows, time_major, rpw);
    } else {
        hipLaunchKernelGGL(gather_rows_kernel<1>, grid, dim3(256), 0, s, table, ids, out, B, T, D, table_rows, time_major, rpw);
    }
    return ds::check_launch("ds_gather_rows");
}

extern "C" int ds_embedding_grad(const float *dx, const int64_t *ids, float *dtable, int32_t B, int32_t T, int32_t D,
                                 int64_t table_rows, int32_t time_major, void *stream) {
    DS_REQUIRE(dx && ids && dtable && B > 0 && T > 0 && D > 0 && D <= 512 && table_rows > 0,
               "ds_embedding_grad: bad argument (D <= 512)");
    const dim3 grid((unsigned)((table_rows + 3) / 4)), block(256);
    hipStream_t s = (hipStream_t)stream;
    if (D <= 64) hipLaunchKernelGGL(embedding_grad_kernel<1>, grid, block, 0, s, dx, ids, dtable, B, T, D, table_rows, time_major);
    else if (D <= 128) hipLaunchKernelGGL(embedding_grad_kernel<2>, grid, block, 0, s, dx, ids, dtable, B, T, D, table_rows, time_major);
    else if (D <= 320) hipLaunchKernelGGL(embedding_grad_kernel<5>, grid, block, 0, s, dx, ids, dtable, B, T, D, table_rows, time_major);
    else hipLaunchKernelGGL(embedding_grad_kernel<8>, grid, block, 0, s, dx, ids, dtable, B, T, D, table_rows, time_major);
    return ds::check_launch("ds_embedding_grad");
}

extern "C" int ds_lstm_cell_fwd(float *gates, const float *rec_slabs, int32_t nslabs, int64_t slab_stride,
                                const float *c_prev, const float *h_prev, const int64_t *seq_len, int32_t t, int32_t B,
                                int32_t H, float forget_bias, float *c_out, float *h_out, void *stream) {
    DS_REQUIRE(gates && c_prev && h_prev && seq_len && c_out && h_out && B > 0 && H > 0 && nslabs >= 0 &&
                   (nslabs == 0 || rec_slabs),
               "ds_lstm_cell_fwd: bad argument");
    hipLaunchKernelGGL(lstm_cell_fwd_kernel, dim3(ds::stream_grid((int64_t)B * H, 256)), dim3(256), 0,
                       (hipStream_t)stream, gates, rec_slabs, nslabs, slab_stride, c_prev, h_prev, seq_len, t, B, H,
                       forget_bias, c_out, h_out);
    return ds::check_launch("ds_lstm_cell_fwd");
}

extern "C" int ds_lstm_cell_bwd(const float *acts, const float *c_t, const float *c_prev, const float *dh,
                                const float *dh_slabs, int32_t nslabs, int64_t slab_stride, const float *dc,
                                const int64_t *seq_len, int32_t t, int32_t B, int32_t H, float *dgates,
                                float *dc_prev, float *dh_carry, void *stream) {
    DS_REQUIRE(acts && c_t && c_prev && dh && dc && seq_len && dgates && dc_prev && dh_carry && nslabs >= 0 &&
                   (nslabs == 0 || dh_slabs),
               "ds_lstm_cell_bwd: bad argument");
    hipLaunchKernelGGL(lstm_cell_bwd_kernel, dim3(ds::stream_grid((int64_t)B * H, 256)), dim3(256), 0,
                       (hipStream_t)stream, acts, c_t, c_prev, dh, dh_slabs, nslabs, slab_stride, dc, seq_len, t, B,
                       H, dgates, dc_prev, dh_carry);
    return ds::check_launch("ds_lstm_cell_bwd");
}

extern "C" int ds_softmax_ce(const float *logits, const int64_t *labels, int32_t B, int32_t C, float grad_scale,
                             const float *grad_scale_dev, float *loss, float *dlogits, void *stream) {
    DS_REQUIRE(logits && labels && B > 0 && C > 0, "ds_softmax_ce: bad argument");
    hipLaunchKernelGGL(softmax_ce_kernel, dim3(1), dim3(256), 0, (hipStream_t)stream, logits, labels, B, C, grad_scale,
                       grad_scale_dev, loss, dlogits);
    return ds::check_launch("ds_softmax_ce");
}

extern "C" int ds_adam_tf(float *theta, const float *g, float *m, float *v, int64_t n, int64_t n_wd, float wd,
                          float grad_scale, float lr_t, const float *lr_t_dev, float beta1, float beta2, float eps,
                          void *stream) {
    DS_REQUIRE(theta && g && m && v && n > 0 && n_wd >= 0 && n_wd <= n, "ds_adam_tf: bad argument");
    hipLaunchKernelGGL(adam_tf_kernel, dim3(ds::stream_grid(n, 256)), dim3(256), 0, (hipStream_t)stream, theta, g, m, v,
                       n, n_wd, wd, grad_scale, lr_t, lr_t_dev, beta1, beta2, eps);
    return ds::check_launch("ds_adam_tf");
}

extern "C" int ds_sumsq(const float *x, int64_t n, float *scratch, float *out, void *stream) {
    DS_REQUIRE(x && scratch && out && n > 0, "ds_sumsq: bad argument");
    int blocks = ds::stream_grid(n, 256 * 8);
    if (blocks > kSumsqBlocks) blocks = kSumsqBlocks;
    hipLaunchKernelGGL(sumsq_stage1, dim3(blocks), dim3(256), 0, (hipStream_t)stream, x, n, scratch);
    hipLaunchKernelGGL(sum_stage2, dim3(1), dim3(256), 0, (hipStream_t)stream, scratch, blocks, out);
    return ds::check_launch("ds_sumsq");
}

__global__ __launch_bounds__(256) void seq_sort_desc_kernel(const int64_t *seq_len, int B, int T, int *perm, int64_t *len_sorted) {
    extern __shared__ int lens[];
    for (int i = threadIdx.x; i < B; i += 256) {
        const int64_t l = seq_len[i];
        lens[i] = (int)(l < 0 ? 0 : (l > T ? T : l));
    }
    __syncthreads();
    for (int i = threadIdx.x; i < B; i += 256) {
        const int li = lens[i];
        int rank = 0;
        for (int j = 0; j < B; ++j) {
            const int lj = lens[j];
            rank += (lj > li || (lj == li && j < i)) ? 1 : 0;
        }
        perm[rank] = i;
        len_sorted[rank] = li;
    }
}

template <typename E>
__global__ __launch_bounds__(256) void permute_rows_kernel(const E *src, int64_t lds, E *dst, int64_t ldd, const int *perm,
                                                           int rows, int cols, int gather) {
    const int64_t total = (int64_t)rows * cols;
    for (int64_t i = (int64_t)blockIdx.x * 256 + threadIdx.x; i < total; i += (int64_t)gridDim.x * 256) {
        const int r = (int)(i / cols), c = (int)(i - (int64_t)r * cols);
        const int pr = perm[r];
        if (gather) dst[(int64_t)r * ldd + c] = src[(int64_t)pr * lds + c];
        else dst[(int64_t)pr * ldd + c] = src[(int64_t)r * lds + c];
    }
}

extern "C" int ds_seq_sort_desc(const int64_t *seq_len, int32_t B, int32_t T, int32_t *perm, int64_t *len_sorted, void *stream) {
    DS_REQUIRE(seq_len && perm && len_sorted && B > 0 && B <= 4096 && T > 0, "ds_seq_sort_desc: bad argument (1 <= B <= 4096)");
    hipLaunchKernelGGL(seq_sort_desc_kernel, dim3(1), dim3(256), (size_t)B * sizeof(int), (hipStream_t)stream, seq_len, B, T, perm,
                       len_sorted);
    return ds::check_launch("ds_seq_sort_desc");
}

extern "C" int ds_permute_rows(const void *src, int64_t lds, void *dst, int64_t ldd, const int32_t *perm, int32_t rows, int32_t cols,
                               int32_t elem_bytes, int32_t gather, void *stream) {
    DS_REQUIRE(src && dst && perm && rows > 0 && cols > 0 && lds >= cols && ldd >= cols && (elem_bytes == 4 || elem_bytes == 8),
               "ds_permute_rows: bad argument (elem_bytes 4 or 8)");
    const int grid = ds::stream_grid((int64_t)rows * cols, 256);
    if (elem_bytes == 4)
        hipLaunchKernelGGL(permute_rows_kernel<float>, dim3(grid), dim3(256), 0, (hipStream_t)stream, (const float *)src, lds,
                           (float *)dst, ldd, perm, rows, cols, gather);
    else
        hipLaunchKernelGGL(permute_rows_kernel<int64_t>, dim3(grid), dim3(256), 0, (hipStream_t)stream, (const int64_t *)src, lds,
                           (int64_t *)dst, ldd, perm, rows, cols, gather);
    return ds::check_launch("ds_permute_rows");
}

extern "C" int ds_colsum(const float *x, int64_t M, int32_t C, int32_t ld, float *scratch, float *out, void *stream) {
    DS_REQUIRE(x && scratch && out && M > 0 && C > 0 && ld >= C, "ds_colsum: bad argument");
    int RS = (int)((M + 63) / 64);
    if (RS > 64) RS = 64;
    const int rps = (int)((M + RS - 1) / RS);
    if (RS <= 8) {
        hipLaunchKernelGGL(colsum_small_kernel, dim3((C + 63) / 64), dim3(256), 0, (hipStream_t)stream, x, M, C, ld, rps, RS, out);
        return ds::check_launch("ds_colsum");
    }
    hipLaunchKernelGGL(colsum_stage1, dim3((C + 63) / 64, RS), dim3(256), 0, (hipStream_t)stream, x, M, C, ld, rps,
                       scratch);
    hipLaunchKernelGGL(colsum_stage2, dim3((C + 255) / 256), dim3(256), 0, (hipStream_t)stream, scratch, RS, C, out);
    return ds::check_launch("ds_colsum");
}

__global__ __launch_bounds__(256) void slab_epilogue_kernel(const float *slabs, int splits, int64_t slab_stride, int lds,
                                                            int64_t M, int N, float *out, int ldo, const float *bias,
                                                            const float *mask, int ldmask, int flags) {
    const int64_t total = M * N;
    for (int64_t i = (int64_t)blockIdx.x * 256 + threadIdx.x; i < total; i += (int64_t)gridDim.x * 256) {
        const int64_t m = i / N;
        const int n = (int)(i - m * N);
        float v = 0.f;
        for (int k = 0; k < splits; ++k) v += slabs[(int64_t)k * slab_stride + m * lds + n];
        if (flags & DS_EPI_BIAS) v += bias[n];
        const int64_t o = m * ldo + n;
        if (flags & DS_EPI_ACCUM) v += out[o];
        if (flags & DS_EPI_MASK) v = mask[m * ldmask + n] > 0.f ? v : 0.f;
        if (flags & DS_EPI_RELU) v = fmaxf(v, 0.f);
        out[o] = v;
    }
}

extern "C" int ds_slab_epilogue(const float *slabs, int32_t splits, int64_t slab_stride, int32_t lds, int64_t M, int32_t N,
                                float *out, int32_t ldo, const float *bias, const float *mask, int32_t ldmask, int32_t flags,
                                void *stream) {
    DS_REQUIRE(slabs && out && splits >= 1 && M > 0 && N > 0 && lds >= N && ldo >= N, "ds_slab_epilogue: bad argument");
    DS_REQUIRE((flags & ~(DS_EPI_BIAS | DS_EPI_ACCUM | DS_EPI_MASK | DS_EPI_RELU)) == 0 && (!(flags & DS_EPI_BIAS) || bias) &&
                   (!(flags & DS_EPI_MASK) || (mask && ldmask >= N)),
               "ds_slab_epilogue: flags are BIAS / ACCUM / MASK / RELU (with their operands)");
    hipLaunchKernelGGL(slab_epilogue_kernel, dim3(ds::stream_grid(M * N, 256)), dim3(256), 0, (hipStream_t)stream, slabs, splits,
                       slab_stride, lds, M, N, out, ldo, bias, mask, ldmask, flags);
    return ds::check_launch("ds_slab_epilogue");
}

extern "C" int ds_copy2d(const float *src, int32_t lds, float *dst, int32_t ldd, int64_t rows, int32_t cols,
                         void *stream) {
    DS_REQUIRE(src && dst && rows > 0 && cols > 0, "ds_copy2d: bad argument");
    hipLaunchKernelGGL(copy2d_kernel, dim3(ds::stream_grid(rows * cols, 256)), dim3(256), 0, (hipStream_t)stream, src,
                       lds, dst, ldd, rows, cols);
    return ds::check_launch("ds_copy2d");
}

extern "C" int ds_pad_channels(const float *src, int32_t cs, float *dst, int32_t cd, int64_t pixels, void *stream) {
    DS_REQUIRE(src && dst && cs > 0 && cd >= cs && pixels > 0, "ds_pad_channels: bad argument");
    hipLaunchKernelGGL(pad_channels_kernel, dim3(ds::stream_grid(pixels * cd, 256)), dim3(256), 0, (hipStream_t)stream,
                       src, cs, dst, cd, pixels);
    return ds::check_launch("ds_pad_channels");
}

extern "C" int ds_fill(float *dst, int64_t n, float value, void *stream) {
    DS_REQUIRE(dst && n > 0, "ds_fill: bad argument");
    hipLaunchKernelGGL(fill_kernel, dim3(ds::stream_grid(n, 256)), dim3(256), 0, (hipStream_t)stream, dst, n, value);
    return ds::check_launch("ds_fill");
}
```

### tumblr_emotions_amd/engine_text.py

```python
import ctypes as C

import torch

from . import _lib, ops
from .ops import WgradPlan, gemm_plan, head_gemm_plan, DS_EPI_ACCUM, DS_EPI_BIAS, DS_EPI_MASK, DS_EPI_RELU

FORGET_BIAS = 1.0


def _vp(addr):
    return C.c_void_p(addr)


def _gemm_wgrad(M, K, N, lda, lddz):
    return WgradPlan(M, 1, 1, K, lda, 1, 1, 1, N, lddz, pad_t=0, pad_l=0, OH=1, OW=1)


class TextTowerEngine:
    KERNEL = "Text/rnn/basic_lstm_cell/kernel"
    BIAS = "Text/rnn/basic_lstm_cell/bias"
    EMB = "Text/W_embedding"

    def __init__(self, store, vocab_rows, embed_dim, rnn_size, post_size, device="cuda", trainable_embedding=False):
        self.store, self.V, self.D, self.H, self.T = store, vocab_rows, embed_dim, rnn_size, post_size
        self.device = torch.device(device)
        self.trainable_embedding = trainable_embedding
        store.declare(self.EMB, (vocab_rows, embed_dim), trainable_embedding, bucket=1)
        store.declare(self.KERNEL, (embed_dim + rnn_size, 4 * rnn_size), True, bucket=1)
        store.declare(self.BIAS, (4 * rnn_size,), True, bucket=1)
        self.B = None
        self.reducer = None
        self.persistent = True
        self.seq_rows = 1
        self.sort_by_length = _lib.tuning_env("DS_LSTM_SORT", "1") != "0" 

    def alloc(self, B):
        if self.B == B:
            return
        dev, T, D, H = self.device, self.T, self.D, self.H
        self.B = B
        self.alloc_gen = getattr(self, "alloc_gen", 0) + 1
        self.use_seq = self.persistent and ops.lstm_seq_supported(B, H)
        self.sorted = bool(self.use_seq and self.sort_by_length)
        if self.sorted:
            self.perm = torch.empty(B, dtype=torch.int32, device=dev)
            self.len_sorted = torch.empty(B, dtype=torch.int64, device=dev)
            self.texts_sorted = torch.empty(B, T, dtype=torch.int64, device=dev)
            self.h_last = torch.empty(B, H, device=dev)
            self.dh_sorted = torch.empty(B, H, device=dev)
        self.seq_ws = torch.zeros(max(ops.lstm_seq_workspace(B, H) // 4, 4), dtype=torch.int32, device=dev)
        self.x = torch.empty(T * B, D, device=dev)
        self.gates = torch.empty(T, B, 4 * H, device=dev)
        self.dgates = torch.empty(T, B, 4 * H, device=dev)
        self.h = torch.zeros(T + 1, B, H, device=dev)
        self.c = torch.zeros(T + 1, B, H, device=dev)
        self.dh = [torch.empty(B, H, device=dev), torch.empty(B, H, device=dev)]
        self.dc = torch.empty(B, H, device=dev)
        st = self.store
        self.table = st.view(self.EMB)
        kptr = st.ptr(self.KERNEL)
        self.wx, self.wh = _vp(kptr), _vp(kptr + 4 * D * 4 * H)
        self.bias = _vp(st.ptr(self.BIAS))
        gk = st.grad_ptr(self.KERNEL)
        self.gwx, self.gwh = _vp(gk), _vp(gk + 4 * D * 4 * H)
        self.gbias = st.grad_view(self.BIAS)
        self.xproj = gemm_plan(T * B, D, 4 * H, D, 4 * H, 4 * H, flags=DS_EPI_BIAS)
        def nsplit(m, n, k):
            blocks = -(-m // 128) * -(-n // 32)
            return int(max(1, min(512 // max(blocks, 1), (k // 16) // 4)))
        self.sf, self.sb = nsplit(B, 4 * H, H), nsplit(B, H, 4 * H)
        self.rec_slabs = torch.empty(self.sf, B, 4 * H, device=dev)
        self.dh_slabs = torch.empty(self.sb, B, H, device=dev)
        self.rec = gemm_plan(B, H, 4 * H, H, 4 * H, 4 * H, splits=self.sf, z_split_stride=B * 4 * H)
        self.rec_dgrad = gemm_plan(B, 4 * H, H, 4 * H, H, 4 * H, transposed_w=True, splits=self.sb,
                                   z_split_stride=B * H)
        self.wgrad_x = _gemm_wgrad(T * B, D, 4 * H, D, 4 * H)
        self.wgrad_h = _gemm_wgrad(T * B, H, 4 * H, H, 4 * H)
        self.ws_bytes = max(self.wgrad_x.ws_bytes, self.wgrad_h.ws_bytes)
        self.ws = torch.empty(max(self.ws_bytes // 4, 4), device=dev)
        self.colsum_scratch = torch.empty(64 * 4 * H, device=dev)
        if self.trainable_embedding:
            self.dx = torch.empty(T * B, D, device=dev)
            self.x_dgrad = gemm_plan(T * B, 4 * H, D, 4 * H, D, 4 * H, transposed_w=True)
            self.gtable = st.grad_view(self.EMB)

    def forward(self, texts, seq_lens):
        B, T, H = texts.shape[0], self.T, self.H
        assert texts.shape[1] == T and texts.dtype == torch.int64 and seq_lens.dtype == torch.int64
        self.alloc(B)
        if self.sorted:
            if not seq_lens.is_contiguous() or not texts.is_contiguous():
                seq_lens, texts = seq_lens.contiguous(), texts.contiguous()
            ops.seq_sort_desc(seq_lens, B, T, self.perm, self.len_sorted)
            ops.permute_rows(texts, self.texts_sorted, self.perm, B, T, gather=True)
            seq_lens, texts = self.len_sorted, self.texts_sorted
        self.seq_lens, self.texts = seq_lens, texts
        ops.gather_rows(self.table, texts, self.x, B, T, self.D, time_major=True)
        self.xproj.run(ops._p(self.x), self.wx, ops._p(self.gates), bias=self.bias)
        if self.use_seq:
            rows = self.seq_rows | (_lib.DS_LSTM_SKIP_MASKED if self.sorted else 0)
            ops.lstm_seq_fwd(self.gates, self.wh, 4 * H, self.h, self.c, seq_lens, T, B, H, FORGET_BIAS, self.seq_ws, rows=rows)
            if self.sorted:
                ops.permute_rows(self.h[T], self.h_last, self.perm, B, H, gather=False)
                return self.h_last
            return self.h[T]
        slab = B * 4 * H
        for t in range(T):
            ns = 0
            if t > 0:
                self.rec.run(ops._p(self.h[t]), self.wh, ops._p(self.rec_slabs))
                ns = self.sf
            ops.lstm_cell_fwd(self.gates[t], self.c[t], self.h[t], seq_lens, t, B, H, FORGET_BIAS, self.c[t + 1],
                              self.h[t + 1], self.rec_slabs, ns, slab)
        return self.h[T]

    def check_status(self):
        if self.B is not None and self.use_seq:
            ops.lstm_seq_status(self.seq_ws, self.B)

    def backward(self, dh_last):
        B, T, H = self.B, self.T, self.H
        if self.use_seq:
            rows = self.seq_rows
            if self.sorted:
                ops.permute_rows(dh_last, self.dh_sorted, self.perm, B, H, gather=True)
                dh_last, rows = self.dh_sorted, rows | _lib.DS_LSTM_SKIP_MASKED
            ops.lstm_seq_bwd(self.gates, self.wh, 4 * H, self.c, dh_last, dh_last.stride(0), self.seq_lens, T, B, H,
                             self.dgates, self.seq_ws, rows=rows)
            return self._weight_grads()
        dh, dh2 = self.dh
        ops.copy2d(dh_last, dh_last.stride(0), dh, H, B, H)
        ops.fill(self.dc, B * H, 0.0)
        ns = 0
        for t in range(T - 1, -1, -1):
            ops.lstm_cell_bwd(self.gates[t], self.c[t + 1], self.c[t], dh, self.dc, self.seq_lens, t, B, H,
                              self.dgates[t], self.dc, dh2, self.dh_slabs, ns, B * H)
            if t > 0:
                self.rec_dgrad.run(ops._p(self.dgates[t]), self.wh, ops._p(self.dh_slabs))
                ns = self.sb
            dh, dh2 = dh2, dh
        self._weight_grads()

    def _weight_grads(self):
        B, T, H = self.B, self.T, self.H
        dg = ops._p(self.dgates)
        self.wgrad_x.run(ops._p(self.x), dg, self.gwx, ops._p(self.ws), self.ws_bytes)
        self.wgrad_h.run(ops._p(self.h), dg, self.gwh, ops._p(self.ws), self.ws_bytes)
        ops.colsum(self.dgates, T * B, 4 * H, 4 * H, self.colsum_scratch, self.gbias)
        if self.trainable_embedding:
            self.x_dgrad.run(dg, self.wx, ops._p(self.dx))
            ops.embedding_grad(self.dx, self.texts, self.gtable, B, T, self.D, time_major=True)
        if self.reducer is not None:
            self.reducer.stage_done("text")


class JointHeadEngine:

    def __init__(self, store, im_size, tx_size, fc_size, nb_emotions, device="cuda"):
        self.store, self.im, self.tx, self.fc, self.nc = store, im_size, tx_size, fc_size, nb_emotions
        self.device = torch.device(device)
        store.declare("W_fc", (im_size + tx_size, fc_size), True, bucket=1)
        store.declare("b_fc", (fc_size,), True, bucket=1)
        store.declare("W_softmax", (fc_size, nb_emotions), True, bucket=1)
        store.declare("b_softmax", (nb_emotions,), True, bucket=1)
        self.B = None
        self.reducer = None

    def alloc(self, B):
        if self.B == B:
            return
        dev, im, tx, fc, nc = self.device, self.im, self.tx, self.fc, self.nc
        self.B = B
        self.alloc_gen = getattr(self, "alloc_gen", 0) + 1
        self.dense = torch.empty(B, fc, device=dev)
        self.ddense = torch.empty(B, fc, device=dev)
        self.logits = torch.empty(B, nc, device=dev)
        self.d_im = torch.empty(B, im, device=dev)
        self.d_tx = torch.empty(B, tx, device=dev)
        st = self.store
        w = st.ptr("W_fc")
        self.w_im, self.w_tx = _vp(w), _vp(w + 4 * im * fc)
        gw = st.grad_ptr("W_fc")
        self.gw_im, self.gw_tx = _vp(gw), _vp(gw + 4 * im * fc)
        self.b_fc, self.gb_fc = _vp(st.ptr("b_fc")), st.grad_view("b_fc")
        self.w_sm, self.gw_sm = _vp(st.ptr("W_softmax")), _vp(st.grad_ptr("W_softmax"))
        self.b_sm, self.gb_sm = _vp(st.ptr("b_softmax")), st.grad_view("b_softmax")
        self.fc_im = None
        self.ws_bytes = 0
        self.colsum_scratch = torch.empty(64 * max(fc, nc), device=dev)

    def _plans(self, ld_im, ld_tx):
        B, im, tx, fc, nc = self.B, self.im, self.tx, self.fc, self.nc
        self.fc_im = head_gemm_plan(B, im, fc, ld_im, fc, fc, device=self.device)
        self.fc_tx = head_gemm_plan(B, tx, fc, ld_tx, fc, fc, flags=DS_EPI_ACCUM | DS_EPI_BIAS | DS_EPI_RELU, device=self.device)
        self.sm = head_gemm_plan(B, fc, nc, fc, nc, nc, flags=DS_EPI_BIAS, device=self.device)
        self.sm_dgrad = head_gemm_plan(B, nc, fc, nc, fc, nc, transposed_w=True, flags=DS_EPI_MASK, ldmask=fc, device=self.device)
        self.sm_wgrad = _gemm_wgrad(B, fc, nc, fc, nc)
        self.im_dgrad = head_gemm_plan(B, fc, im, fc, im, fc, transposed_w=True, device=self.device)
        self.tx_dgrad = head_gemm_plan(B, fc, tx, fc, tx, fc, transposed_w=True, device=self.device)
        self.im_wgrad = _gemm_wgrad(B, im, fc, ld_im, fc)
        self.tx_wgrad = _gemm_wgrad(B, tx, fc, ld_tx, fc)
        self.ws_bytes = max(p.ws_bytes for p in (self.sm_wgrad, self.im_wgrad, self.tx_wgrad))
        self.ws = torch.empty(max(self.ws_bytes // 4, 4), device=self.device)
        self._lds = (ld_im, ld_tx)

    def forward(self, im_feat, tx_feat):
        B = im_feat.shape[0]
        self.alloc(B)
        lds = (im_feat.stride(0), tx_feat.stride(0))
        if self.fc_im is None or self._lds != lds:
            self._plans(*lds)
        self.im_feat, self.tx_feat = im_feat, tx_feat
        self.fc_im.run(ops._p(im_feat), self.w_im, ops._p(self.dense))
        self.fc_tx.run(ops._p(tx_feat), self.w_tx, ops._p(self.dense), bias=self.b_fc)
        self.sm.run(ops._p(self.dense), self.w_sm, ops._p(self.logits), bias=self.b_sm)
        return self.logits

    def backward(self, dlogits):
        B, fc, nc = self.B, self.fc, self.nc
        dl, ws = ops._p(dlogits), ops._p(self.ws)
        self.sm_wgrad.run(ops._p(self.dense), dl, self.gw_sm, ws, self.ws_bytes)
        ops.colsum(dlogits, B, nc, nc, self.colsum_scratch, self.gb_sm)
        self.sm_dgrad.run(dl, self.w_sm, ops._p(self.ddense), mask=ops._p(self.dense))
        dd = ops._p(self.ddense)
        self.im_wgrad.run(ops._p(self.im_feat), dd, self.gw_im, ws, self.ws_bytes)
        self.tx_wgrad.run(ops._p(self.tx_feat), dd, self.gw_tx, ws, self.ws_bytes)
        ops.colsum(self.ddense, B, fc, fc, self.colsum_scratch, self.gb_fc)
        self.im_dgrad.run(dd, self.w_im, ops._p(self.d_im))
        self.tx_dgrad.run(dd, self.w_tx, ops._p(self.d_tx))
        if self.reducer is not None:
            self.reducer.stage_done("head")
        return self.d_im, self.d_tx

    def input_backward(self, dlogits):
        self.sm_dgrad.run(ops._p(dlogits), self.w_sm, ops._p(self.ddense), mask=ops._p(self.dense))
        self.im_dgrad.run(ops._p(self.ddense), self.w_im, ops._p(self.d_im))
        return self.d_im


class TextHeadEngine:

    def __init__(self, store, rnn_size, nb_emotions, device="cuda"):
        self.store, self.H, self.nc = store, rnn_size, nb_emotions
        self.device = torch.device(device)
        store.declare("W_softmax", (rnn_size, nb_emotions), True, bucket=1)
        store.declare("b_softmax", (nb_emotions,), True, bucket=1)
        self.B = None
        self.reducer = None

    def alloc(self, B):
        if self.B == B:
            return
        dev, H, nc = self.device, self.H, self.nc
        self.B = B
        self.alloc_gen = getattr(self, "alloc_gen", 0) + 1
        self.logits = torch.empty(B, nc, device=dev)
        self.d_tx = torch.empty(B, H, device=dev)
        st = self.store
        self.w_sm, self.gw_sm = _vp(st.ptr("W_softmax")), _vp(st.grad_ptr("W_softmax"))
        self.b_sm, self.gb_sm = _vp(st.ptr("b_softmax")), st.grad_view("b_softmax")
        self.sm = head_gemm_plan(B, H, nc, H, nc, nc, flags=DS_EPI_BIAS, device=self.device)
        self.sm_dgrad = head_gemm_plan(B, nc, H, nc, H, nc, transposed_w=True, device=self.device)
        self.sm_wgrad = _gemm_wgrad(B, H, nc, H, nc)
        self.ws_bytes = self.sm_wgrad.ws_bytes
        self.ws = torch.empty(max(self.ws_bytes // 4, 4), device=dev)
        self.colsum_scratch = torch.empty(64 * max(nc, 4), device=dev)

    def forward(self, tx_feat):
        self.alloc(tx_feat.shape[0])
        assert tx_feat.stride(0) == self.H
        self.tx_feat = tx_feat
        self.sm.run(ops._p(tx_feat), self.w_sm, ops._p(self.logits), bias=self.b_sm)
        return self.logits

    def backward(self, dlogits):
        dl = ops._p(dlogits)
        self.sm_wgrad.run(ops._p(self.tx_feat), dl, self.gw_sm, ops._p(self.ws), self.ws_bytes)
        ops.colsum(dlogits, self.B, self.nc, self.nc, self.colsum_scratch, self.gb_sm)
        self.sm_dgrad.run(dl, self.w_sm, ops._p(self.d_tx))
        if self.reducer is not None:
            self.reducer.stage_done("head")
        return self.d_tx
```

### tumblr_emotions_amd/ops.py

```python
import ctypes as C
import os

import torch

from . import _lib
from ._lib import (ConvDesc, Segments, SumSegments, DS_EPI_ACCUM, DS_EPI_BIAS, DS_EPI_BNSUMS, DS_EPI_MASK, DS_EPI_RELU,
                   DS_EPI_STATS,
                   DS_DTYPE_BF16, DS_DTYPE_F32, DS_FP8_E4M3, DS_FP8_E5M2, DS_CONV_FWD, DS_CONV_DGRAD, DS_ARITH_F32, DS_ARITH_BF16,
                   DS_ARITH_FP8, DS_ARITH_F32X3, DS_FAM_IGEMM, DS_FAM_WINO2, DS_FAM_WINO4, DS_FAM_STEM, DS_FAM_BF16D, DS_FAM_FP8D,
                   DS_FAM_F32X3, DS_FAM_WINO4H, DS_FAM_STEM_POOL, DS_FAM_STEM_DGRAD, DS_PLAN_STEM_POOL, DS_PLAN_NO_SPLITK, DS_PLAN_NO_WINO4H, DS_PLAN_NO_WINO, DS_PLAN_NO_WINO4, DS_PLAN_NO_STEM_DIRECT, DS_PLAN_NO_BF16_DIRECT, DS_PLAN_ACT16,
                   DS_PLAN_PACKED_RGB, DS_PLAN_FP8_EVERYWHERE, DS_PLAN_FP8_WIDE_RULE)


_raw_stream = getattr(torch._C, "_cuda_getCurrentRawStream", None)


def _stream():
    if _raw_stream is not None:
        return C.c_void_p(_raw_stream(torch.cuda.current_device()))
    return C.c_void_p(torch.cuda.current_stream().cuda_stream)


def _p(t):
    if t is None:
        return None
    if not t.is_cuda:
        raise RuntimeError("tumblr_emotions_amd kernels need CUDA/HIP tensors; there is no CPU fallback")
    return C.c_void_p(t.data_ptr())


def same_pad(n, k, s):
    out = -(-n // s)
    total = max((out - 1) * s + k - n, 0)
    return out, total // 2


def make_segments(entries):
    sg = Segments()
    sg.nseg = len(entries)
    for i, e in enumerate(entries):
        c0, c1, ptr, ld = e[:4]
        sg.c_begin[i], sg.c_end[i], sg.ld[i] = c0, c1, ld
        sg.ptr[i] = ptr
        sg.dtype[i] = e[4] if len(e) > 4 else DS_DTYPE_F32
        sg.amax[i] = e[5] if len(e) > 5 else None
    return sg


def act_dtype(t):
    return DS_DTYPE_BF16 if t.dtype == torch.bfloat16 else DS_DTYPE_F32


class ConvPlan:

    def __init__(self, N, H, W, Cin, ldx, KH, KW, stride, Cout, ldz, w_tap_stride, w_n_stride, w_k_stride,
                 flip=0, fold_cin=0, flags=0, ldmask=0, pad_t=None, pad_l=None, OH=None, OW=None,
                 splits=1, z_split_stride=0, dtype=DS_DTYPE_F32):
        d = ConvDesc()
        d.dtype = dtype
        d.N, d.H, d.W, d.Cin, d.ldx = N, H, W, Cin, ldx
        d.KH, d.KW, d.stride = KH, KW, stride
        if OH is None:
            OH, pt = same_pad(H, KH, stride)
            OW, pl = same_pad(W, KW if not fold_cin else (Cin // fold_cin), stride)
            pad_t = pt if pad_t is None else pad_t
            pad_l = pl if pad_l is None else pad_l
        d.pad_t, d.pad_l, d.OH, d.OW = pad_t, pad_l, OH, OW
        d.Cout, d.ldz = Cout, ldz
        d.w_tap_stride, d.w_n_stride, d.w_k_stride = w_tap_stride, w_n_stride, w_k_stride
        d.flip, d.fold_cin, d.flags, d.ldmask = flip, fold_cin, flags, ldmask
        d.splits, d.z_split_stride = splits, z_split_stride
        self.d = d
        self.M = N * OH * OW
        self.partials = _lib.load().ds_conv_igemm_partials(C.byref(d)) if flags & (DS_EPI_STATS | DS_EPI_BNSUMS) else 0
        d.partials = self.partials
        k_alg = KH * KW * Cin if not fold_cin else KH * (Cin // fold_cin) * 3
        self.alg_flops = 2.0 * self.M * Cout * k_alg

    def enable_bnsums(self, ldy):
        if not _lib.load().ds_conv_igemm_bnsums_supported(C.byref(self.d)):
            return 0
        self.d.partials = 0
        self.d.flags |= DS_EPI_BNSUMS
        self.d.ldmask = ldy
        self.partials = _lib.load().ds_conv_igemm_partials(C.byref(self.d))
        self.d.partials = self.partials
        return self.partials

    def run(self, x, w, z, bias=None, mask=None, stats=None, pivot=None):
        t = CONV_TIMER
        if t is not None:
            t.begin()
        _lib.check(_lib.load().ds_conv_igemm(C.byref(self.d), x, w, z, bias, mask, stats, pivot, _stream()),
                   "ds_conv_igemm")
        if t is not None:
            t.end(self)


class ConvTimer:

    def __init__(self):
        self.records = []
        self._start = None

    def begin(self):
        self._start = torch.cuda.Event(enable_timing=True)
        self._start.record(torch.cuda.current_stream())

    def end(self, plan):
        e = torch.cuda.Event(enable_timing=True)
        e.record(torch.cuda.current_stream())
        d = getattr(plan, "d", None)
        pooled = getattr(plan, "family", None) == DS_FAM_STEM_POOL or bool(getattr(d, "pool_argmax", None))
        self.records.append((self._start, e, plan.alg_flops, pooled))

    def summary(self, pooled=None):
        recs = [r for r in self.records if pooled is None or r[3] == pooled]
        ms = sum(s.elapsed_time(e) for (s, e, _, _) in recs)
        return len(recs), ms, sum(f for (_, _, f, _) in recs)


CONV_TIMER = None


def head_gemm_plan(M, K, N, lda, ldc, w_ld, transposed_w=False, flags=0, ldmask=0, *, device):
    if M <= 512 and K >= 256 and _lib.tuning_env("DS_SPLIT_GEMM", "1") != "0":
        return SplitGemm(M, K, N, lda, ldc, w_ld, transposed_w, flags, ldmask, 8 if K >= 512 else 4, device)
    return gemm_plan(M, K, N, lda, ldc, w_ld, transposed_w=transposed_w, flags=flags, ldmask=ldmask)


def gemm_plan(M, K, N, lda, ldc, w_ld, transposed_w=False, flags=0, ldmask=0, splits=1, z_split_stride=0,
              dtype=DS_DTYPE_F32):
    if transposed_w:
        return ConvPlan(M, 1, 1, K, lda, 1, 1, 1, N, ldc, 0, w_ld, 1, flags=flags, ldmask=ldmask,
                        pad_t=0, pad_l=0, OH=1, OW=1, splits=splits, z_split_stride=z_split_stride, dtype=dtype)
    return ConvPlan(M, 1, 1, K, lda, 1, 1, 1, N, ldc, 0, 1, w_ld, flags=flags, ldmask=ldmask,
                    pad_t=0, pad_l=0, OH=1, OW=1, splits=splits, z_split_stride=z_split_stride, dtype=dtype)


class SplitGemm:

    def __init__(self, M, K, N, lda, ldc, w_ld, transposed_w, flags, ldmask, splits, device):
        self.M, self.N, self.ldc, self.flags, self.ldmask, self.splits = M, N, ldc, flags, ldmask, splits
        self.slabs = torch.empty(splits, M, N, device=device)
        self.plan = gemm_plan(M, K, N, lda, N, w_ld, transposed_w=transposed_w, splits=splits, z_split_stride=M * N)
        self.d, self.alg_flops, self.partials = self.plan.d, self.plan.alg_flops, 0

    def run(self, x, w, z, bias=None, mask=None, stats=None, pivot=None):
        if stats is not None or pivot is not None:
            raise ValueError("SplitGemm has no BatchNorm-statistics epilogue (the heads' GEMMs are not followed by BatchNorm)")
        t = CONV_TIMER
        if t is not None:
            t.begin()
        lib = _lib.load()
        _lib.check(lib.ds_conv_igemm(C.byref(self.plan.d), x, w, _p(self.slabs), None, None, None, None, _stream()),
                   "ds_conv_igemm")
        _lib.check(lib.ds_slab_epilogue(_p(self.slabs), self.splits, self.M * self.N, self.N, self.M, self.N, z, self.ldc,
                                        bias, mask, self.ldmask, self.flags, _stream()), "ds_slab_epilogue")
        if t is not None:
            t.end(self)


class WinoPlan:

    def __init__(self, N, H, W, Cin, ldx, Cout, ldz, flags=0, f4=False):
        self.args = (N, H, W, Cin, ldx, Cout, ldz)
        self.flags = flags
        self.f4 = bool(f4)
        lib = _lib.load()
        self._run, self._name = (lib.ds_conv_wino4, "ds_conv_wino4") if f4 else (lib.ds_conv_wino, "ds_conv_wino")
        self._partials = lib.ds_conv_wino4_partials if f4 else lib.ds_conv_wino_partials
        self.u_elems = (36 if f4 else 16) * Cin * Cout
        self.M = N * H * W
        self.partials = self._partials(N, H, W) if flags & (DS_EPI_STATS | DS_EPI_BNSUMS) else 0
        self.alg_flops = 2.0 * self.M * Cout * 9 * Cin

    def enable_bnsums(self):
        N, H, W = self.args[:3]
        self.flags = (self.flags & ~DS_EPI_STATS) | DS_EPI_BNSUMS
        self.partials = self._partials(N, H, W)
        return self.partials

    def set_ldx(self, ldx):
        self.args = self.args[:4] + (ldx,) + self.args[5:]

    def set_ldz(self, ldz):
        self.args = self.args[:6] + (ldz,)

    def run(self, x, u, z, stats=None, pivot=None, ymask=None):
        t = CONV_TIMER
        if t is not None:
            t.begin()
        N, H, W, Cin, ldx, Cout, ldz = self.args
        _lib.check(self._run(x, u, z, stats, pivot, ymask, N, H, W, Cin, ldx, Cout, ldz, self.flags, _stream()), self._name)
        if t is not None:
            t.end(self)


class LayerPlan:

    def __init__(self, role, arith, options, N, H, W, w_cin, w_cout, k, stride, ldx, ldz, flags=0):
        self.p = _lib.LayerPlanStruct()
        _lib.check(_lib.load().ds_conv_plan(C.byref(self.p), role, arith, options, N, H, W, w_cin, w_cout, k, stride, ldx,
                                            ldz, flags), "ds_conv_plan")
        self.d = self.p.d
        self.family = self.p.family
        self.M = N * self.d.OH * self.d.OW
        self.alg_flops = self.p.alg_flops
        self.u = None
        self.wscale = None
        self.io = _lib.ConvIO()
        self.ws_bytes = int(self.p.ws_bytes)
        self.splitk = int(self.p.splitk)
        self._ws = None
        self._run = _lib.load().ds_conv_run
        self._ref = C.byref(self.p)
        self._io_ref = C.byref(self.io)

    @property
    def partials(self):
        return self.p.partials

    @property
    def x16_ok(self):
        return bool(self.p.x16_ok)

    def alloc_weights(self, device):
        if self.p.w_bytes:
            self.u = torch.empty(self.p.w_bytes, dtype=torch.uint8, device=device)
        if self.p.wscale_floats:
            self.wscale = torch.zeros(self.p.wscale_floats, device=device)
            self.io.wscale = self.wscale.data_ptr()

    def set_workspace(self, t):
        assert t.numel() * t.element_size() >= self.ws_bytes
        self._ws = t
        self.io.ws, self.io.ws_bytes = t.data_ptr(), t.numel() * t.element_size()

    def prepare(self, w_hwio):
        if self.u is not None:
            _lib.check(_lib.load().ds_conv_prepare_weights(self._ref, w_hwio, _p(self.u), _p(self.wscale), _stream()),
                       "ds_conv_prepare_weights")

    def enable_bnsums(self, ldy):
        return int(_lib.load().ds_conv_plan_enable_bnsums(self._ref, ldy))

    def norm_supported(self):
        return bool(_lib.load().ds_conv_plan_norm_supported(self._ref))

    def enable_pool3(self, argmax):
        if not _lib.load().ds_conv_plan_enable_pool3(self._ref, _p(argmax)):
            return False
        self.pool_argmax = argmax
        return True

    def finalize_tickets(self):
        return int(_lib.load().ds_conv_plan_finalize_tickets(self._ref))

    def enable_bn_backward_on_load(self, mean, rstd, shift, coef, parts):
        if not _lib.load().ds_conv_plan_bnb_supported(self._ref) or len(parts) > 3:
            return False
        if any(c0 % 16 for (c0, _, _, _) in parts):
            return False
        b = _lib.BnBwdOnLoad()
        b.mean, b.rstd, b.shift, b.coef = mean.data_ptr(), rstd.data_ptr(), shift.data_ptr(), coef.data_ptr()
        b.nseg = len(parts)
        for i, (c0, c1, ptr, ld) in enumerate(parts):
            assert c0 == (parts[i - 1][1] if i else 0)
            b.c_end[i], b.ld[i], b.dy[i] = c1, ld, ptr
        self.bnb = b
        self.d.bnb = C.addressof(b)
        return True

    def run(self, x, w_hwio, z, stats=None, pivot=None, mask=None, bias=None, x_amax=None, fin=None):
        t = CONV_TIMER
        if t is not None:
            t.begin()
        io = self.io
        io.stats, io.pivot, io.mask, io.bias, io.x_amax, io.fin = stats, pivot, mask, bias, x_amax, fin
        _lib.check(self._run(self._ref, x, w_hwio if self.u is None else self.u.data_ptr(), z, self._io_ref, _stream()),
                   "ds_conv_run")
        if t is not None:
            t.end(self)


def conv_norm_supported(plan):
    return bool(_lib.load().ds_conv_igemm_norm_supported(C.byref(plan.d)))


def wino4_supported(H, W, Cin, Cout):
    return bool(_lib.load().ds_conv_wino4_supported(H, W, Cin, Cout))


def wino4_prefer(N, H, W, Cin, Cout):
    return bool(_lib.load().ds_conv_wino4_prefer(N, H, W, Cin, Cout))


def wino_transform_weights(w_ptr, u, Cin, Cout, dgrad, f4=False):
    lib = _lib.load()
    if f4:
        _lib.check(lib.ds_wino4_transform_weights(w_ptr, _p(u), Cin, Cout, int(dgrad), _stream()), "ds_wino4_transform_weights")
    else:
        _lib.check(lib.ds_wino_transform_weights(w_ptr, _p(u), Cin, Cout, int(dgrad), _stream()), "ds_wino_transform_weights")


class StemPlan:

    def __init__(self, N, H, W, cin_store, Cout, ldz, bf16=False):
        self.args = (N, H, W, cin_store, Cout, ldz)
        self.bf16 = bf16
        self.flags = DS_EPI_STATS
        OH, OW = (H + 1) // 2, (W + 1) // 2
        self.M = N * OH * OW
        self.partials = (_lib.load().ds_conv_stem_bf16_partials if bf16 else _lib.load().ds_conv_stem_partials)(N, OH, OW)
        self.alg_flops = 2.0 * self.M * Cout * 147

    def run(self, x, w, z, stats=None, pivot=None):
        t = CONV_TIMER
        if t is not None:
            t.begin()
        N, H, W, cs, Cout, ldz = self.args
        f = _lib.load().ds_conv_stem_bf16 if self.bf16 else _lib.load().ds_conv_stem
        _lib.check(f(x, w, z, stats, pivot, N, H, W, cs, Cout, ldz, _stream()), "ds_conv_stem")
        if t is not None:
            t.end(self)


class Bf16Plan:

    def __init__(self, N, H, W, Cin, ldx, k, stride, Cout, ldz, flags=0, pad_t=None, pad_l=None, OH=None, OW=None):
        d = ConvDesc()
        d.dtype = DS_DTYPE_BF16
        d.N, d.H, d.W, d.Cin, d.ldx = N, H, W, Cin, ldx
        d.KH, d.KW, d.stride = k, k, stride
        if OH is None:
            OH, pt = same_pad(H, k, stride)
            OW, pl = same_pad(W, k, stride)
            pad_t = pt if pad_t is None else pad_t
            pad_l = pl if pad_l is None else pad_l
        d.pad_t, d.pad_l, d.OH, d.OW = pad_t, pad_l, OH, OW
        d.Cout, d.ldz, d.flags, d.splits = Cout, ldz, flags, 1
        self.d = d
        lib = _lib.load()
        if not lib.ds_conv_bf16_supported(C.byref(d)):
            raise ValueError("ds_conv_bf16 does not take this geometry")
        self.M = N * OH * OW
        self.partials = lib.ds_conv_bf16_partials(C.byref(d)) if flags & DS_EPI_STATS else 0
        self.alg_flops = 2.0 * self.M * Cout * k * k * Cin

    def set_ldx(self, ldx):
        self.d.ldx = ldx

    @property
    def flags(self):
        return self.d.flags

    @flags.setter
    def flags(self, v):
        self.d.flags = v

    def run(self, x, wb, z, stats=None, pivot=None, mask=None):
        t = CONV_TIMER
        if t is not None:
            t.begin()
        _lib.check(_lib.load().ds_conv_bf16(C.byref(self.d), x, wb, z, mask, stats, pivot, _stream()), "ds_conv_bf16")
        if t is not None:
            t.end(self)


class Fp8Plan(Bf16Plan):

    def __init__(self, N, H, W, Cin, ldx, k, stride, Cout, ldz, flags=0, a_format=DS_FP8_E4M3, **kw):
        super().__init__(N, H, W, Cin, ldx, k, stride, Cout, ldz, flags=flags, **kw)
        lib = _lib.load()
        if not lib.ds_conv_fp8_supported(C.byref(self.d)):
            raise ValueError("ds_conv_fp8 does not take this geometry")
        self.a_format = a_format
        self.partials = lib.ds_conv_fp8_partials(C.byref(self.d)) if flags & DS_EPI_STATS else 0

    def run(self, x, wq, z, stats=None, pivot=None, x_amax=None, wscale=None, mask=None):
        t = CONV_TIMER
        if t is not None:
            t.begin()
        _lib.check(_lib.load().ds_conv_fp8(C.byref(self.d), x, x_amax, self.a_format, wq, wscale, z, mask, stats, pivot,
                                           _stream()), "ds_conv_fp8")
        if t is not None:
            t.end(self)


AMAX_FLOATS = 512
WSCALE_FLOATS = 4 + AMAX_FLOATS


def amax_value(record):
    return float(record.view(-1)[:AMAX_FLOATS:32].max().item())


def absmax(x, n, out, x_dtype=DS_DTYPE_F32):
    if not isinstance(x, C.c_void_p):
        x_dtype = act_dtype(x)
        x = _p(x)
    _lib.check(_lib.load().ds_absmax(x, n, x_dtype, _p(out), _stream()), "ds_absmax")


def weights_fp8_bytes(Cin, Cout, taps, dgrad):
    return int(_lib.load().ds_weights_fp8_bytes(Cin, Cout, taps, int(dgrad)))


def weights_to_fp8(w_ptr, wq, wscale, Cin, Cout, taps, dgrad):
    _lib.check(_lib.load().ds_weights_to_fp8(w_ptr, _p(wq), _p(wscale), Cin, Cout, taps, int(dgrad), _stream()),
               "ds_weights_to_fp8")


def weights_bf16_bytes(Cin, Cout, taps, dgrad):
    return int(_lib.load().ds_weights_bf16_bytes(Cin, Cout, taps, int(dgrad)))


def weights_to_bf16(w_ptr, wb, Cin, Cout, taps, dgrad):
    _lib.check(_lib.load().ds_weights_to_bf16(w_ptr, _p(wb), Cin, Cout, taps, int(dgrad), _stream()),
               "ds_weights_to_bf16")


class F32x3Plan:
    f4 = False

    def __init__(self, N, H, W, Cin, ldx, k, stride, Cout, ldz, flags=0, pad_t=None, pad_l=None, OH=None, OW=None):
        d = ConvDesc()
        d.dtype = DS_DTYPE_F32
        d.N, d.H, d.W, d.Cin, d.ldx = N, H, W, Cin, ldx
        d.KH, d.KW, d.stride = k, k, stride
        if OH is None:
            OH, pt = same_pad(H, k, stride)
            OW, pl = same_pad(W, k, stride)
            pad_t = pt if pad_t is None else pad_t
            pad_l = pl if pad_l is None else pad_l
        d.pad_t, d.pad_l, d.OH, d.OW = pad_t, pad_l, OH, OW
        d.Cout, d.ldz, d.flags, d.splits = Cout, ldz, flags, 1
        self.d = d
        lib = _lib.load()
        if not lib.ds_conv_f32x3_supported(C.byref(d)):
            raise ValueError("ds_conv_f32x3 does not take this geometry")
        self.M = N * OH * OW
        self.partials = lib.ds_conv_f32x3_partials(C.byref(d)) if flags & DS_EPI_STATS else 0
        self.partials_for_sums = lib.ds_conv_f32x3_partials(C.byref(d))
        self.alg_flops = 2.0 * self.M * Cout * k * k * Cin

    def set_ldx(self, ldx):
        self.d.ldx = ldx

    def set_ldz(self, ldz):
        self.d.ldz = ldz

    @property
    def flags(self):
        return self.d.flags

    @flags.setter
    def flags(self, v):
        self.d.flags = v

    def run(self, x, wb, z, stats=None, pivot=None, mask=None):
        t = CONV_TIMER
        if t is not None:
            t.begin()
        _lib.check(_lib.load().ds_conv_f32x3(C.byref(self.d), x, wb, z, mask, stats, pivot, _stream()), "ds_conv_f32x3")
        if t is not None:
            t.end(self)


def weights_f32x3_bytes(Cin, Cout, taps, dgrad):
    return int(_lib.load().ds_weights_f32x3_bytes(Cin, Cout, taps, int(dgrad)))


def weights_to_f32x3(w_ptr, wb, Cin, Cout, taps, dgrad):
    _lib.check(_lib.load().ds_weights_to_f32x3(w_ptr, _p(wb), Cin, Cout, taps, int(dgrad), _stream()), "ds_weights_to_f32x3")


class WgradPlan:

    def __init__(self, N, H, W, Cin, ldx, KH, KW, stride, Cout, lddz, pad_t=None, pad_l=None, OH=None, OW=None,
                 fold_cin=0):
        d = ConvDesc()
        d.fold_cin = fold_cin
        d.N, d.H, d.W, d.Cin, d.ldx = N, H, W, Cin, ldx
        d.KH, d.KW, d.stride = KH, KW, stride
        if OH is None:
            OH, pad_t = same_pad(H, KH, stride)
            OW, pad_l = same_pad(W, KW if not fold_cin else Cin // fold_cin, stride)
        d.pad_t, d.pad_l, d.OH, d.OW = pad_t, pad_l, OH, OW
        d.Cout, d.ldz = Cout, Cout
        self.d = d
        self.lddz = lddz
        self.ws_bytes = int(_lib.load().ds_conv_wgrad_workspace(C.byref(d)))

    def run(self, x, dz, dw, ws, ws_bytes):
        _lib.check(_lib.load().ds_conv_wgrad(C.byref(self.d), x, dz, self.lddz, dw, ws, ws_bytes, _stream()),
                   "ds_conv_wgrad")


def bn_finalize(stats, P, count, C_, beta, eps, decay, mean, rstd, shift, mm, mv, pivot=None):
    _lib.check(_lib.load().ds_bn_finalize(_p(stats), P, count, C_, _p(beta), _p(pivot), eps, decay, _p(mean),
                                          _p(rstd), _p(shift), _p(mm), _p(mv), _stream()), "ds_bn_finalize")


def bn_finalize_centered(stats, P, count, C_, beta, eps, decay, mean, rstd, shift, mm, mv, pivot, mean_c, shift_c):
    _lib.check(_lib.load().ds_bn_finalize_centered(_p(stats), P, count, C_, _p(beta), _p(pivot), eps, decay, _p(mean), _p(rstd),
                                                   _p(shift), _p(mm), _p(mv), _p(mean_c), _p(shift_c), _stream()),
               "ds_bn_finalize_centered")


def bn_apply_relu(z, M, C_, rstd, shift, segs):
    if z.dtype == torch.bfloat16:
        _lib.check(_lib.load().ds_bn_apply_relu_z16(_p(z), M, C_, _p(rstd), _p(shift), C.byref(segs), _stream()),
                   "ds_bn_apply_relu_z16")
        return
    _lib.check(_lib.load().ds_bn_apply_relu(_p(z), M, C_, _p(rstd), _p(shift), C.byref(segs), _stream()),
               "ds_bn_apply_relu")


def bn_infer_prepare(beta, mm, mv, eps, C_, rstd, shift):
    _lib.check(_lib.load().ds_bn_infer_prepare(_p(beta), _p(mm), _p(mv), eps, C_, _p(rstd), _p(shift), _stream()),
               "ds_bn_infer_prepare")


def bn_bwd_partials(M, C_):
    return _lib.load().ds_bn_bwd_partials(M, C_)


def bn_bwd_reduce(z, segs, M, C_, mean, rstd, shift, partials, ldz=None, z_dtype=DS_DTYPE_F32):
    ptr = lambda t: t if isinstance(t, C.c_void_p) else _p(t)
    if not isinstance(z, C.c_void_p):
        z_dtype = act_dtype(z)
    _lib.check(_lib.load().ds_bn_bwd_reduce(ptr(z), C_ if ldz is None else ldz, z_dtype, C.byref(segs), M, C_, ptr(mean),
                                            ptr(rstd), ptr(shift), ptr(partials), _stream()), "ds_bn_bwd_reduce")


def bn_bwd_finalize_segs(sum_segs, M, C_, beta, dbeta, coef):
    _lib.check(_lib.load().ds_bn_bwd_finalize_segs(C.byref(sum_segs), M, C_, _p(beta), _p(dbeta), _p(coef), _stream()),
               "ds_bn_bwd_finalize_segs")


class BnFinalizeJobs:

    def __init__(self, jobs):
        self.n = len(jobs)
        self.arr = (_lib.BnFinalizeJob * self.n)()
        self._keep = jobs
        for a, (stats, P, count, C_, beta, pivot, mean, rstd, shift, mm, mv) in zip(self.arr, jobs):
            a.stats, a.P, a.C, a.count = stats.data_ptr(), P, C_, count
            a.beta, a.pivot = beta.data_ptr(), (pivot.data_ptr() if pivot is not None else None)
            a.mean, a.rstd, a.shift = mean.data_ptr(), rstd.data_ptr(), shift.data_ptr()
            a.moving_mean = mm.data_ptr() if mm is not None else None
            a.moving_var = mv.data_ptr() if mv is not None else None

    def run(self, eps, decay):
        _lib.check(_lib.load().ds_bn_finalize_multi(C.cast(self.arr, C.c_void_p), self.n, eps, decay, _stream()),
                   "ds_bn_finalize_multi")


def bn_bwd_finalize_multi(sum_segs, M, C_, betas, dbetas, coef):
    n = sum_segs.nseg
    b = (C.c_void_p * 4)(*[t.data_ptr() for t in betas[:n]])
    d = (C.c_void_p * 4)(*[(t.data_ptr() if t is not None else None) for t in dbetas[:n]])
    _lib.check(_lib.load().ds_bn_bwd_finalize_multi(C.byref(sum_segs), M, C_, C.cast(b, C.c_void_p), C.cast(d, C.c_void_p),
                                                    _p(coef), _stream()), "ds_bn_bwd_finalize_multi")


def bn_finalize_apply_relu(stats, P, count, C_, beta, eps, decay, mean, rstd, shift, mm, mv, pivot, z, M, segs, ticket):
    _lib.check(_lib.load().ds_bn_finalize_apply_relu(_p(stats), P, count, C_, _p(beta), _p(pivot), eps, decay, _p(mean), _p(rstd),
                                                     _p(shift), _p(mm), _p(mv), _p(z), M, C.byref(segs), _p(ticket), _stream()),
               "ds_bn_finalize_apply_relu")


def bn_bwd_finalize_apply(sum_segs, M, C_, beta, dbeta, coef, z, segs, mean, rstd, shift, dz, ticket, amax=None, ldz=0,
                          betas=None, dbetas=None):
    bv = dv = None
    if betas is not None:
        n = sum_segs.nseg
        bv = C.cast((C.c_void_p * 4)(*[t.data_ptr() for t in betas[:n]]), C.c_void_p)
        dv = C.cast((C.c_void_p * 4)(*[(t.data_ptr() if t is not None else None) for t in dbetas[:n]]), C.c_void_p)
    out16 = dz.dtype == torch.bfloat16
    _lib.check(_lib.load().ds_bn_bwd_finalize_apply(C.byref(sum_segs), _p(beta), _p(dbeta), bv, dv, _p(coef), _p(z), ldz or C_,
                                                    C.byref(segs), M, C_, _p(mean), _p(rstd), _p(shift), _p(dz),
                                                    DS_DTYPE_BF16 if out16 else DS_DTYPE_F32, dz.stride(0) if out16 else 0,
                                                    _p(amax), _p(ticket), _stream()), "ds_bn_bwd_finalize_apply")


def bn_bwd_finalize(partials, P, M, C_, dbeta, coef):
    _lib.check(_lib.load().ds_bn_bwd_finalize(_p(partials), P, M, C_, _p(dbeta), _p(coef), _stream()),
               "ds_bn_bwd_finalize")


def bn_bwd_apply(z, segs, M, C_, mean, rstd, shift, coef, dz, amax=None, ldz=0):
    if z.dtype == torch.bfloat16:
        assert dz.dtype == torch.bfloat16
        _lib.check(_lib.load().ds_bn_bwd_apply_z16(_p(z), ldz or C_, C.byref(segs), M, C_, _p(mean), _p(rstd), _p(shift),
                                                   _p(coef), _p(dz), dz.stride(0), _p(amax), _stream()), "ds_bn_bwd_apply_z16")
        return
    if dz.dtype == torch.bfloat16:
        _lib.check(_lib.load().ds_bn_bwd_apply_bf16(_p(z), ldz or C_, C.byref(segs), M, C_, _p(mean), _p(rstd), _p(shift),
                                                    _p(coef), _p(dz), dz.stride(0), _p(amax), _stream()), "ds_bn_bwd_apply_bf16")
        return
    _lib.check(_lib.load().ds_bn_bwd_apply(_p(z), ldz or C_, C.byref(segs), M, C_, _p(mean), _p(rstd), _p(shift), _p(coef),
                                           _p(dz), _p(amax), _stream()), "ds_bn_bwd_apply")


def maxpool_fwd(x, y, argmax, N, H, W, C_, k, stride, mode="SAME"):
    if mode == "SAME":
        OH, pt = same_pad(H, k, stride)
        OW, pl = same_pad(W, k, stride)
    else:
        OH, OW, pt, pl = (H - k) // stride + 1, (W - k) // stride + 1, 0, 0
    assert x.dtype == y.dtype
    _lib.check(_lib.load().ds_maxpool_fwd(_p(x), _p(y), _p(argmax), N, H, W, C_, k, stride, pt, pl, OH, OW,
                                          act_dtype(x), _stream()), "ds_maxpool_fwd")
    return OH, OW


def maxpool_bn_relu_fwd(z, rstd, shift, y, argmax, N, H, W, C_, k, stride, amax=None):
    OH, pt = same_pad(H, k, stride)
    OW, pl = same_pad(W, k, stride)
    _lib.check(_lib.load().ds_maxpool_bn_relu_fwd(_p(z), _p(rstd), _p(shift), _p(y), _p(argmax), N, H, W, C_, k, stride,
                                                  pt, pl, OH, OW, act_dtype(y), _p(amax), _stream()),
               "ds_maxpool_bn_relu_fwd")
    return OH, OW


def bn_pool_bwd_partials(N, H, W, C_):
    OH, _ = same_pad(H, 3, 2)
    OW, _ = same_pad(W, 3, 2)
    return _lib.load().ds_bn_pool_bwd_partials(N, OH, OW, C_)


def bn_pool_bwd_reduce(z, dpool, argmax, N, H, W, C_, mean, rstd, shift, partials):
    OH, pt = same_pad(H, 3, 2)
    OW, pl = same_pad(W, 3, 2)
    _lib.check(_lib.load().ds_bn_pool_bwd_reduce(_p(z), _p(dpool), _p(argmax), N, H, W, C_, pt, pl, OH, OW, _p(mean),
                                                 _p(rstd), _p(shift), _p(partials), _stream()), "ds_bn_pool_bwd_reduce")


def bn_pool_bwd_apply(z, dpool, argmax, N, H, W, C_, mean, rstd, shift, coef, dz):
    OH, pt = same_pad(H, 3, 2)
    OW, pl = same_pad(W, 3, 2)
    _lib.check(_lib.load().ds_bn_pool_bwd_apply(_p(z), _p(dpool), _p(argmax), N, H, W, C_, pt, pl, OH, OW, _p(mean),
                                                _p(rstd), _p(shift), _p(coef), _p(dz), _stream()), "ds_bn_pool_bwd_apply")


def maxpool_bwd(dy, argmax, dx, accumulate, N, H, W, C_, k, stride, mode="SAME"):
    if dy.dtype == torch.bfloat16:
        assert k == 3 and stride == 1 and mode == "SAME"
        _lib.check(_lib.load().ds_maxpool3_bwd_dy16(_p(dy), _p(argmax), _p(dx), int(accumulate), None, DS_DTYPE_F32, N, H, W, C_,
                                                    None, _stream()), "ds_maxpool3_bwd_dy16")
        return
    if mode == "SAME":
        OH, pt = same_pad(H, k, stride)
        OW, pl = same_pad(W, k, stride)
    else:
        OH, OW, pt, pl = (H - k) // stride + 1, (W - k) // stride + 1, 0, 0
    _lib.check(_lib.load().ds_maxpool_bwd(_p(dy), _p(argmax), _p(dx), int(accumulate), N, H, W, C_, k, stride, pt,
                                          pl, OH, OW, _stream()), "ds_maxpool_bwd")


def maxpool3_bwd_sums_partials(N, W, C_):
    return _lib.load().ds_maxpool3_bwd_sums_partials(N, W, C_)


def maxpool3_bwd_sums(dy, argmax, dx, accumulate, y, N, H, W, C_, partials):
    if dy.dtype == torch.bfloat16:
        _lib.check(_lib.load().ds_maxpool3_bwd_dy16(_p(dy), _p(argmax), _p(dx), int(accumulate), _p(y), act_dtype(y), N, H, W, C_,
                                                    _p(partials), _stream()), "ds_maxpool3_bwd_dy16")
        return
    _lib.check(_lib.load().ds_maxpool3_bwd_sums(_p(dy), _p(argmax), _p(dx), int(accumulate), _p(y), act_dtype(y), N, H, W, C_,
                                                _p(partials), _stream()), "ds_maxpool3_bwd_sums")


def avgpool_dropout_fwd(x, N, HW, C_, keep, seed, mask_in, mask_out, out, seed_dev=None):
    _lib.check(_lib.load().ds_avgpool_dropout_fwd(_p(x), N, HW, C_, keep, seed, _p(seed_dev), _p(mask_in),
                                                  _p(mask_out), _p(out), _stream()), "ds_avgpool_dropout_fwd")


def avgpool_dropout_bwd(dout, mask, N, HW, C_, keep, dx):
    _lib.check(_lib.load().ds_avgpool_dropout_bwd(_p(dout), _p(mask), N, HW, C_, keep, _p(dx), _stream()),
               "ds_avgpool_dropout_bwd")


def gather_rows(table, ids, out, B, T, D, time_major=True):
    _lib.check(_lib.load().ds_gather_rows(_p(table), _p(ids), _p(out), B, T, D, table.shape[0], int(time_major),
                                          _stream()), "ds_gather_rows")


def embedding_grad(dx, ids, dtable, B, T, D, time_major=True):
    _lib.check(_lib.load().ds_embedding_grad(_p(dx), _p(ids), _p(dtable), B, T, D, dtable.shape[0], int(time_major),
                                             _stream()), "ds_embedding_grad")


def lstm_cell_fwd(gates, c_prev, h_prev, seq_len, t, B, H, forget_bias, c_out, h_out, rec_slabs=None, nslabs=0,
                  slab_stride=0):
    _lib.check(_lib.load().ds_lstm_cell_fwd(_p(gates), _p(rec_slabs), nslabs, slab_stride, _p(c_prev), _p(h_prev),
                                            _p(seq_len), t, B, H, forget_bias, _p(c_out), _p(h_out), _stream()),
               "ds_lstm_cell_fwd")


def lstm_cell_bwd(acts, c_t, c_prev, dh, dc, seq_len, t, B, H, dgates, dc_prev, dh_carry, dh_slabs=None, nslabs=0,
                  slab_stride=0):
    _lib.check(_lib.load().ds_lstm_cell_bwd(_p(acts), _p(c_t), _p(c_prev), _p(dh), _p(dh_slabs), nslabs, slab_stride,
                                            _p(dc), _p(seq_len), t, B, H, _p(dgates), _p(dc_prev), _p(dh_carry),
                                            _stream()), "ds_lstm_cell_bwd")


def lstm_seq_supported(B, H):
    return bool(_lib.load().ds_lstm_seq_supported(B, H))


def lstm_seq_workspace(B, H):
    return int(_lib.load().ds_lstm_seq_workspace(B, H))


def lstm_seq_fwd(gates, wh_ptr, ldw, h, c, seq_len, T, B, H, forget_bias, ws, rows=1):
    _lib.check(_lib.load().ds_lstm_seq_fwd(_p(gates), wh_ptr, ldw, _p(h), _p(c), _p(seq_len), T, B, H, forget_bias,
                                           int(rows), _p(ws), ws.numel() * ws.element_size(), _stream()),
               "ds_lstm_seq_fwd")


def lstm_seq_bwd(acts, wh_ptr, ldw, c, dh_last, ld_dh, seq_len, T, B, H, dgates, ws, rows=1):
    _lib.check(_lib.load().ds_lstm_seq_bwd(_p(acts), wh_ptr, ldw, _p(c), _p(dh_last), ld_dh, _p(seq_len), T, B, H,
                                           _p(dgates), int(rows), _p(ws), ws.numel() * ws.element_size(), _stream()),
               "ds_lstm_seq_bwd")


def seq_sort_desc(seq_len, B, T, perm, len_sorted):
    _lib.check(_lib.load().ds_seq_sort_desc(_p(seq_len), B, T, _p(perm), _p(len_sorted), _stream()), "ds_seq_sort_desc")


def permute_rows(src, dst, perm, rows, cols, gather=True):
    assert src.element_size() == dst.element_size() and src.element_size() in (4, 8)
    _lib.check(_lib.load().ds_permute_rows(_p(src), src.stride(0), _p(dst), dst.stride(0), _p(perm), rows, cols, src.element_size(),
                                           int(bool(gather)), _stream()), "ds_permute_rows")


def lstm_seq_status(ws, B):
    rc = _lib.load().ds_lstm_seq_status(_p(ws), B)
    if rc != 0:
        which = " and ".join(n for b, n in ((1, "forward"), (2, "backward")) if rc > 0 and rc & b) or "status read"
        raise RuntimeError("ds_lstm_seq: a workgroup hand-off of the %s launch timed out (status %d): the LSTM results "
                           "of this step are invalid (a workgroup of a row group never became resident)" % (which, rc))
    return rc


def softmax_ce(logits, labels, B, C_, grad_scale, grad_scale_dev, loss, dlogits):
    _lib.check(_lib.load().ds_softmax_ce(_p(logits), _p(labels), B, C_, grad_scale, _p(grad_scale_dev), _p(loss),
                                         _p(dlogits), _stream()), "ds_softmax_ce")


def adam_tf(theta, g, m, v, n, n_wd, wd, grad_scale, lr_t, b1, b2, eps, lr_t_dev=None):
    _lib.check(_lib.load().ds_adam_tf(_p(theta), _p(g), _p(m), _p(v), n, n_wd, wd, grad_scale, lr_t, _p(lr_t_dev),
                                      b1, b2, eps, _stream()), "ds_adam_tf")


def sumsq(x, n, scratch, out):
    _lib.check(_lib.load().ds_sumsq(_p(x), n, _p(scratch), _p(out), _stream()), "ds_sumsq")


def colsum(x, M, C_, ld, scratch, out):
    _lib.check(_lib.load().ds_colsum(_p(x), M, C_, ld, _p(scratch), _p(out), _stream()), "ds_colsum")


def copy2d(src, lds, dst, ldd, rows, cols):
    _lib.check(_lib.load().ds_copy2d(_p(src), lds, _p(dst), ldd, rows, cols, _stream()), "ds_copy2d")


def pad_channels(src, cs, dst, cd, pixels):
    _lib.check(_lib.load().ds_pad_channels(_p(src), cs, _p(dst), cd, pixels, _stream()), "ds_pad_channels")


def fill(dst, n, value):
    _lib.check(_lib.load().ds_fill(_p(dst), n, value, _stream()), "ds_fill")
```

Before: 19560 samples/s.

## Skip padded timesteps in LSTM weight-gradient GEMMs and bias colsum

With sequences sorted by length, the sort kernel now also builds a per-timestep prefix count of active rows. The LSTM input and recurrent weight-gradient kernels and the bias column-sum read this prefix on the device and reduce only over rows that are still active, so the zero gradient rows past each sequence's end are never read. Work is split by the packed row count rather than T*B. In exchange the inner loop does extra index mapping and a small prefix walk, and correctness relies on dgates being zero for masked rows.

```diff
diff --git a/include/ds_kernels.h b/include/ds_kernels.h
--- a/include/ds_kernels.h
+++ b/include/ds_kernels.h
@@ -232,6 +232,8 @@
 size_t ds_conv_wgrad_workspace(const ds_conv_desc *d);
 int ds_conv_wgrad(const ds_conv_desc *d, const float *x, const float *dz, int32_t lddz, float *dw,
                   void *ws, size_t ws_bytes, void *stream);
+int ds_conv_wgrad_rows(const ds_conv_desc *d, const float *x, const float *dz, int32_t lddz, float *dw, void *ws,
+                       size_t ws_bytes, const int32_t *row_prefix, int32_t T, void *stream);
 
 int ds_bn_finalize(const float *stats, int32_t P, int64_t count, int32_t C, const float *beta, const float *pivot,
                    float eps, float decay, float *mean, float *rstd, float *shift, float *moving_mean,
@@ -352,6 +354,8 @@
                      float *dh_carry, void *stream);
 
 int ds_seq_sort_desc(const int64_t *seq_len, int32_t B, int32_t T, int32_t *perm, int64_t *len_sorted, void *stream);
+int ds_seq_sort_desc_rows(const int64_t *seq_len, int32_t B, int32_t T, int32_t *perm, int64_t *len_sorted, int32_t *row_prefix,
+                          void *stream);
 int ds_permute_rows(const void *src, int64_t lds, void *dst, int64_t ldd, const int32_t *perm, int32_t rows, int32_t cols,
                     int32_t elem_bytes, int32_t gather, void *stream);
 #define DS_LSTM_SKIP_MASKED 256
@@ -377,6 +381,8 @@
 
 int ds_sumsq(const float *x, int64_t n, float *scratch, float *out, void *stream);
 int ds_colsum(const float *x, int64_t M, int32_t C, int32_t ld, float *scratch, float *out, void *stream);
+int ds_colsum_rows(const float *x, int32_t T, int32_t B, int32_t C, int32_t ld, const int32_t *row_prefix, float *scratch,
+                   float *out, void *stream);
 int ds_slab_epilogue(const float *slabs, int32_t splits, int64_t slab_stride, int32_t lds, int64_t M, int32_t N, float *out,
                      int32_t ldo, const float *bias, const float *mask, int32_t ldmask, int32_t flags, void *stream);
 int ds_copy2d(const float *src, int32_t lds, float *dst, int32_t ldd, int64_t rows, int32_t cols,
diff --git a/tumblr_emotions_amd/_lib.py b/tumblr_emotions_amd/_lib.py
--- a/tumblr_emotions_amd/_lib.py
+++ b/tumblr_emotions_amd/_lib.py
@@ -147,6 +147,7 @@
     "ds_conv_run": (C.c_int, [_LP, _P, _P, _P, _IO, _P]),
     "ds_conv_wgrad_workspace": (C.c_size_t, [_CD]),
     "ds_conv_wgrad": (C.c_int, [_CD, _P, _P, _i32, _P, _P, C.c_size_t, _P]),
+    "ds_conv_wgrad_rows": (C.c_int, [_CD, _P, _P, _i32, _P, _P, C.c_size_t, _P, _i32, _P]),
     "ds_bn_finalize": (C.c_int, [_P, _i32, _i64, _i32, _P, _P, _f32, _f32, _P, _P, _P, _P, _P, _P]),
     "ds_bn_finalize_centered": (C.c_int, [_P, _i32, _i64, _i32, _P, _P, _f32, _f32, _P, _P, _P, _P, _P, _P, _P, _P]),
     "ds_bn_apply_relu": (C.c_int, [_P, _i64, _i32, _P, _P, _SG, _P]),
@@ -179,6 +180,7 @@
     "ds_lstm_cell_fwd": (C.c_int, [_P, _P, _i32, _i64, _P, _P, _P, _i32, _i32, _i32, _f32, _P, _P, _P]),
     "ds_lstm_cell_bwd": (C.c_int, [_P, _P, _P, _P, _P, _i32, _i64, _P, _P, _i32, _i32, _i32, _P, _P, _P, _P]),
     "ds_seq_sort_desc": (C.c_int, [_P, _i32, _i32, _P, _P, _P]),
+    "ds_seq_sort_desc_rows": (C.c_int, [_P, _i32, _i32, _P, _P, _P, _P]),
     "ds_permute_rows": (C.c_int, [_P, _i64, _P, _i64, _P, _i32, _i32, _i32, _i32, _P]),
     "ds_lstm_seq_supported": (C.c_int, [_i32, _i32]),
     "ds_lstm_seq_workspace": (C.c_size_t, [_i32, _i32]),
@@ -189,6 +191,7 @@
     "ds_adam_tf": (C.c_int, [_P, _P, _P, _P, _i64, _i64, _f32, _f32, _f32, _P, _f32, _f32, _f32, _P]),
     "ds_sumsq": (C.c_int, [_P, _i64, _P, _P, _P]),
     "ds_colsum": (C.c_int, [_P, _i64, _i32, _i32, _P, _P, _P]),
+    "ds_colsum_rows": (C.c_int, [_P, _i32, _i32, _i32, _i32, _P, _P, _P, _P]),
     "ds_slab_epilogue": (C.c_int, [_P, _i32, _i64, _i32, _i64, _i32, _P, _i32, _P, _P, _i32, _i32, _P]),
     "ds_copy2d": (C.c_int, [_P, _i32, _P, _i32, _i64, _i32, _P]),
     "ds_pad_channels": (C.c_int, [_P, _i32, _P, _i32, _i64, _P]),
diff --git a/tumblr_emotions_amd/csrc/conv_wgrad.hip b/tumblr_emotions_amd/csrc/conv_wgrad.hip
--- a/tumblr_emotions_amd/csrc/conv_wgrad.hip
+++ b/tumblr_emotions_amd/csrc/conv_wgrad.hip
@@ -24,9 +24,12 @@
     unsigned x_bytes, z_bytes;
     float inv_ohw, inv_ow;
     int slabs;
+    const int *row_prefix;
+    int rows_T, rows_B;
 };
 
 constexpr unsigned kOOB = 0x80000000u;
+constexpr int kMaxPackedT = 1024;
 
 __device__ __forceinline__ __amdgpu_buffer_rsrc_t make_srd(const void *p, unsigned bytes) {
     return __builtin_amdgcn_make_buffer_rsrc(const_cast<void *>(p), 0, (int)bytes, 0x00020000);
@@ -197,10 +200,11 @@
     return v;
 }
 
-template <int AI, int BJ>
+template <int AI, int BJ, bool PACKED = false>
 __global__ __launch_bounds__(256, (AI * BJ > 8) ? 1 : 2) void wgrad_direct_kernel(const WgradParams p) {
     constexpr int NACC = AI * BJ, U = DS_WG_U;
     __shared__ __attribute__((aligned(16))) float red[2 * NACC * 16 * 64];
+    __shared__ int pre_s[PACKED ? kMaxPackedT + 1 : 1];
     const ds_conv_desc &d = p.d;
     const int tid = threadIdx.x, lane = tid & 63;
     const int wave = __builtin_amdgcn_readfirstlane(tid >> 6);
@@ -218,9 +222,16 @@
     const __amdgpu_buffer_rsrc_t srd_x = make_srd(p.x, p.x_bytes);
     const __amdgpu_buffer_rsrc_t srd_z = make_srd(p.dz, p.z_bytes);
 
-    const int m_begin = split * p.pix_per_split;
-    int m_end = m_begin + p.pix_per_split;
-    if (m_end > p.M) m_end = p.M;
+    int M = p.M, pps = p.pix_per_split;
+    if constexpr (PACKED) {
+        for (int i = tid; i <= p.rows_T; i += 256) pre_s[i] = p.row_prefix[i];
+        __syncthreads();
+        M = pre_s[p.rows_T];
+        pps = ((M + p.slabs - 1) / p.slabs + 7) / 8 * 8;
+    }
+    const int m_begin = split * pps;
+    int m_end = m_begin + pps;
+    if (m_end > M) m_end = M;
     int q = (m_end - m_begin + 3) / 4;
     q = (q + 1) & ~1;
     const int wb = m_begin + wave * q;
@@ -232,7 +243,12 @@
     const int ohw = d.OH * d.OW;
     int oh = 0, ow = 0;
     unsigned offx, offz;
-    {
+    int pt = 0, pc = 0, pn = 0;
+    if constexpr (PACKED) {
+        pc = pre_s[0];
+        pn = pre_s[1];
+        offx = offz = 0;
+    } else {
         const int mm = m < p.M ? m : 0;
         const int n = mm / ohw;
         const int r = mm - n * ohw;
@@ -259,6 +275,18 @@
     const int OWc = d.OW, OHc = d.OH;
     auto offsets = [&](unsigned &ox, unsigned &oz) {
         const bool mv = m < we;
+        if constexpr (PACKED) {
+            while (m >= pn && pt < p.rows_T - 1) {
+                ++pt;
+                pc = pn;
+                pn = pre_s[pt + 1];
+            }
+            const unsigned row = (unsigned)(pt * p.rows_B + (m - pc));
+            oz = (mv && co_ok) ? (row * (unsigned)p.lddz + (unsigned)co) * 4u : kOOB;
+            ox = (mv && ci_ok) ? (row * (unsigned)d.ldx + (unsigned)ci) * 4u : kOOB;
+            m += 2;
+            return;
+        }
         const bool in = (unsigned)(oh - lo_h) <= span_h && (unsigned)(ow - lo_w) <= span_w;
         oz = (mv && co_ok) ? offz : kOOB;
         ox = (mv && ci_ok && in) ? offx : kOOB;
@@ -488,8 +516,10 @@
     return (size_t)splits * d->KH * d->KW * d->Cin * d->Cout * sizeof(float);
 }
 
-extern "C" int ds_conv_wgrad(const ds_conv_desc *d, const float *x, const float *dz, int32_t lddz, float *dw,
-                             void *ws, size_t ws_bytes, void *stream) {
+namespace {
+
+int wgrad_launch(const ds_conv_desc *d, const float *x, const float *dz, int32_t lddz, float *dw, void *ws, size_t ws_bytes,
+                 const int32_t *row_prefix, int32_t T, void *stream) {
     DS_REQUIRE(d && x && dz && dw, "ds_conv_wgrad: null argument");
     const int64_t M = (int64_t)d->N * d->OH * d->OW;
     DS_REQUIRE(M < (1ll << 31), "ds_conv_wgrad: M too large");
@@ -507,6 +537,9 @@
     }
     WgradParams p;
     p.d = *d;
+    p.row_prefix = row_prefix;
+    p.rows_T = T;
+    p.rows_B = row_prefix ? (int)(M / T) : 0;
     p.x = x; p.dz = dz; p.lddz = lddz;
     p.out = splits == 1 ? dw : (float *)ws;
     p.M = (int)M;
@@ -527,7 +560,11 @@
         const int co_tiles = (d->Cout + 32 * pl.bj - 1) / (32 * pl.bj);
         p.slabs = splits;
         const dim3 grid((unsigned)(d->KH * d->KW * p.ci_tiles * co_tiles * splits));
-#define DS_WG(A, B) if (pl.ai == A && pl.bj == B) hipLaunchKernelGGL((wgrad_direct_kernel<A, B>), grid, dim3(256), 0, s, p);
+#define DS_WG(A, B)                                                                                   \
+    if (pl.ai == A && pl.bj == B) {                                                                   \
+        if (row_prefix) hipLaunchKernelGGL((wgrad_direct_kernel<A, B, true>), grid, dim3(256), 0, s, p); \
+        else hipLaunchKernelGGL((wgrad_direct_kernel<A, B>), grid, dim3(256), 0, s, p);                 \
+    }
         DS_WG(4, 4) DS_WG(4, 2) DS_WG(4, 1) DS_WG(2, 4) DS_WG(2, 2) DS_WG(2, 1) DS_WG(1, 4) DS_WG(1, 2) DS_WG(1, 1)
 #undef DS_WG
     } else {
@@ -545,3 +582,20 @@
     }
     return ds::check_launch("ds_conv_wgrad");
 }
+
+}
+
+extern "C" int ds_conv_wgrad(const ds_conv_desc *d, const float *x, const float *dz, int32_t lddz, float *dw,
+                             void *ws, size_t ws_bytes, void *stream) {
+    return wgrad_launch(d, x, dz, lddz, dw, ws, ws_bytes, nullptr, 0, stream);
+}
+
+extern "C" int ds_conv_wgrad_rows(const ds_conv_desc *d, const float *x, const float *dz, int32_t lddz, float *dw, void *ws,
+                                  size_t ws_bytes, const int32_t *row_prefix, int32_t T, void *stream) {
+    DS_REQUIRE(d && row_prefix && T > 0 && T <= kMaxPackedT && d->N % T == 0, "ds_conv_wgrad_rows: bad argument (1 <= T <= 1024, "
+               "T divides the rows)");
+    DS_REQUIRE(d->H == 1 && d->W == 1 && d->OH == 1 && d->OW == 1 && d->KH == 1 && d->KW == 1 && d->stride == 1 && d->pad_t == 0 &&
+                   d->pad_l == 0 && d->fold_cin == 0,
+               "ds_conv_wgrad_rows: GEMM geometry only (H = W = OH = OW = KH = KW = stride = 1, no padding)");
+    return wgrad_launch(d, x, dz, lddz, dw, ws, ws_bytes, row_prefix, T, stream);
+}
diff --git a/tumblr_emotions_amd/csrc/text_misc.hip b/tumblr_emotions_amd/csrc/text_misc.hip
--- a/tumblr_emotions_amd/csrc/text_misc.hip
+++ b/tumblr_emotions_amd/csrc/text_misc.hip
@@ -319,6 +319,73 @@
     out[c] = (float)acc;
 }
 
+constexpr int kColsumRS = 64;
+typedef float f32x4 __attribute__((ext_vector_type(4)));
+
+__global__ __launch_bounds__(256) void colsum_rows_stage1(const float *__restrict__ x, int T, int B, int C, int ld,
+                                                          const int *__restrict__ row_prefix, float *__restrict__ partials) {
+    __shared__ f32x4 red[4][64];
+    const int lane = threadIdx.x & 63, wave = threadIdx.x >> 6;
+    const int c = blockIdx.x * 256 + lane * 4;
+    const int S = min(row_prefix[T], T * B);
+    const int per = (S + kColsumRS - 1) / kColsumRS;
+    const int p0 = blockIdx.y * per;
+    const int p1 = p0 + per < S ? p0 + per : S;
+    f32x4 acc = {0.f, 0.f, 0.f, 0.f};
+    if (p0 + wave < p1) {
+        int t = 0, pc = row_prefix[0], pn = row_prefix[1];
+        auto row_of = [&](int p) {
+            while (p >= pn && t < T - 1) {
+                ++t;
+                pc = pn;
+                pn = row_prefix[t + 1];
+            }
+            return (int64_t)t * B + (p - pc);
+        };
+        constexpr int U = 4;
+        for (int p = p0 + wave; p < p1; p += 4 * U) {
+            f32x4 v[U];
+#pragma unroll
+            for (int u = 0; u < U; ++u) {
+                const int pu = p + 4 * u;
+                v[u] = f32x4{0.f, 0.f, 0.f, 0.f};
+                if (pu < p1) {
+                    const int64_t m = row_of(pu);
+                    if (c < C && m < (int64_t)T * B) v[u] = *reinterpret_cast<const f32x4 *>(x + m * ld + c);
+                }
+            }
+#pragma unroll
+            for (int u = 0; u < U; ++u) acc += v[u];
+        }
+    }
+    red[wave][lane] = acc;
+    __syncthreads();
+    if (wave == 0 && c < C)
+        *reinterpret_cast<f32x4 *>(partials + (int64_t)blockIdx.y * C + c) = ((red[0][lane] + red[1][lane]) + red[2][lane]) + red[3][lane];
+}
+
+__global__ __launch_bounds__(256) void colsum_rows_stage2(const float *__restrict__ partials, int C, float *__restrict__ out) {
+    __shared__ f32x4 red[16][16];
+    const int cl = threadIdx.x & 15, sl = threadIdx.x >> 4;
+    const int c = blockIdx.x * 64 + cl * 4;
+    f32x4 v[kColsumRS / 16];
+#pragma unroll
+    for (int k = 0; k < kColsumRS / 16; ++k)
+        v[k] = c < C ? *reinterpret_cast<const f32x4 *>(partials + (int64_t)(sl + 16 * k) * C + c) : f32x4{0.f, 0.f, 0.f, 0.f};
+    f32x4 acc = v[0];
+#pragma unroll
+    for (int k = 1; k < kColsumRS / 16; ++k) acc += v[k];
+    red[sl][cl] = acc;
+    __syncthreads();
+    if (sl == 0 && c < C) {
+        f32x4 s = red[0][cl];
+#pragma unroll
+        for (int k = 1; k < 16; ++k) s += red[k][cl];
+#pragma unroll
+        for (int e = 0; e < 4; ++e) out[c + e] = s[e];
+    }
+}
+
 __global__ __launch_bounds__(256) void copy2d_kernel(const float *src, int lds, float *dst, int ldd, int64_t rows,
                                                      int cols) {
     const int64_t total = rows * cols;
@@ -445,13 +512,28 @@
     return ds::check_launch("ds_sumsq");
 }
 
-__global__ __launch_bounds__(256) void seq_sort_desc_kernel(const int64_t *seq_len, int B, int T, int *perm, int64_t *len_sorted) {
+__global__ __launch_bounds__(256) void seq_sort_desc_kernel(const int64_t *seq_len, int B, int T, int *perm, int64_t *len_sorted,
+                                                            int *row_prefix) {
     extern __shared__ int lens[];
+    int *hist = lens + B;
+    if (row_prefix)
+        for (int t = threadIdx.x; t <= T; t += 256) hist[t] = 0;
+    __syncthreads();
     for (int i = threadIdx.x; i < B; i += 256) {
         const int64_t l = seq_len[i];
         lens[i] = (int)(l < 0 ? 0 : (l > T ? T : l));
-    }
-    __syncthreads();
+        if (row_prefix) atomicAdd(&hist[lens[i]], 1);
+    }
+    __syncthreads();
+    if (row_prefix && threadIdx.x == 0) {
+        int acc = 0, le = 0;
+        for (int t = 0; t < T; ++t) {
+            row_prefix[t] = acc;
+            le += hist[t];
+            acc += B - le;
+        }
+        row_prefix[T] = acc;
+    }
     for (int i = threadIdx.x; i < B; i += 256) {
         const int li = lens[i];
         int rank = 0;
@@ -479,8 +561,17 @@
 extern "C" int ds_seq_sort_desc(const int64_t *seq_len, int32_t B, int32_t T, int32_t *perm, int64_t *len_sorted, void *stream) {
     DS_REQUIRE(seq_len && perm && len_sorted && B > 0 && B <= 4096 && T > 0, "ds_seq_sort_desc: bad argument (1 <= B <= 4096)");
     hipLaunchKernelGGL(seq_sort_desc_kernel, dim3(1), dim3(256), (size_t)B * sizeof(int), (hipStream_t)stream, seq_len, B, T, perm,
-                       len_sorted);
+                       len_sorted, (int *)nullptr);
     return ds::check_launch("ds_seq_sort_desc");
+}
+
+extern "C" int ds_seq_sort_desc_rows(const int64_t *seq_len, int32_t B, int32_t T, int32_t *perm, int64_t *len_sorted,
+                                     int32_t *row_prefix, void *stream) {
+    DS_REQUIRE(seq_len && perm && len_sorted && row_prefix && B > 0 && B <= 4096 && T > 0 && T <= 4096,
+               "ds_seq_sort_desc_rows: bad argument (1 <= B <= 4096, 1 <= T <= 4096)");
+    hipLaunchKernelGGL(seq_sort_desc_kernel, dim3(1), dim3(256), (size_t)(B + T + 1) * sizeof(int), (hipStream_t)stream, seq_len, B, T,
+                       perm, len_sorted, row_prefix);
+    return ds::check_launch("ds_seq_sort_desc_rows");
 }
 
 extern "C" int ds_permute_rows(const void *src, int64_t lds, void *dst, int64_t ldd, const int32_t *perm, int32_t rows, int32_t cols,
@@ -510,6 +601,18 @@
                        scratch);
     hipLaunchKernelGGL(colsum_stage2, dim3((C + 255) / 256), dim3(256), 0, (hipStream_t)stream, scratch, RS, C, out);
     return ds::check_launch("ds_colsum");
+}
+
+extern "C" int ds_colsum_rows(const float *x, int32_t T, int32_t B, int32_t C, int32_t ld, const int32_t *row_prefix,
+                              float *scratch, float *out, void *stream) {
+    DS_REQUIRE(x && row_prefix && scratch && out && T > 0 && B > 0 && C > 0 && ld >= C,
+               "ds_colsum_rows: bad argument");
+    DS_REQUIRE(C % 4 == 0 && ld % 4 == 0 && ((uintptr_t)x & 15) == 0 && ((uintptr_t)scratch & 15) == 0,
+               "ds_colsum_rows: C and ld multiples of 4, x and scratch 16-byte aligned");
+    hipLaunchKernelGGL(colsum_rows_stage1, dim3((C + 255) / 256, kColsumRS), dim3(256), 0, (hipStream_t)stream, x, T, B, C, ld,
+                       (const int *)row_prefix, scratch);
+    hipLaunchKernelGGL(colsum_rows_stage2, dim3((C + 63) / 64), dim3(256), 0, (hipStream_t)stream, (const float *)scratch, C, out);
+    return ds::check_launch("ds_colsum_rows");
 }
 
 __global__ __launch_bounds__(256) void slab_epilogue_kernel(const float *slabs, int splits, int64_t slab_stride, int lds,
diff --git a/tumblr_emotions_amd/engine_text.py b/tumblr_emotions_amd/engine_text.py
--- a/tumblr_emotions_amd/engine_text.py
+++ b/tumblr_emotions_amd/engine_text.py
@@ -33,6 +33,7 @@
         self.persistent = True
         self.seq_rows = 1
         self.sort_by_length = _lib.tuning_env("DS_LSTM_SORT", "1") != "0" 
+        self.skip_padding = _lib.tuning_env("DS_TEXT_SKIP_PADDING", "1") != "0"
 
     def alloc(self, B):
         if self.B == B:
@@ -48,6 +49,7 @@
             self.texts_sorted = torch.empty(B, T, dtype=torch.int64, device=dev)
             self.h_last = torch.empty(B, H, device=dev)
             self.dh_sorted = torch.empty(B, H, device=dev)
+            self.row_prefix = torch.zeros(T + 1, dtype=torch.int32, device=dev) if self.skip_padding else None
         self.seq_ws = torch.zeros(max(ops.lstm_seq_workspace(B, H) // 4, 4), dtype=torch.int32, device=dev)
         self.x = torch.empty(T * B, D, device=dev)
         self.gates = torch.empty(T, B, 4 * H, device=dev)
@@ -79,6 +81,7 @@
         self.ws_bytes = max(self.wgrad_x.ws_bytes, self.wgrad_h.ws_bytes)
         self.ws = torch.empty(max(self.ws_bytes // 4, 4), device=dev)
         self.colsum_scratch = torch.empty(64 * 4 * H, device=dev)
+        self.rows_skipped = self.sorted and self.skip_padding
         if self.trainable_embedding:
             self.dx = torch.empty(T * B, D, device=dev)
             self.x_dgrad = gemm_plan(T * B, 4 * H, D, 4 * H, D, 4 * H, transposed_w=True)
@@ -91,7 +94,7 @@
         if self.sorted:
             if not seq_lens.is_contiguous() or not texts.is_contiguous():
                 seq_lens, texts = seq_lens.contiguous(), texts.contiguous()
-            ops.seq_sort_desc(seq_lens, B, T, self.perm, self.len_sorted)
+            ops.seq_sort_desc(seq_lens, B, T, self.perm, self.len_sorted, self.row_prefix)
             ops.permute_rows(texts, self.texts_sorted, self.perm, B, T, gather=True)
             seq_lens, texts = self.len_sorted, self.texts_sorted
         self.seq_lens, self.texts = seq_lens, texts
@@ -144,9 +147,14 @@
     def _weight_grads(self):
         B, T, H = self.B, self.T, self.H
         dg = ops._p(self.dgates)
-        self.wgrad_x.run(ops._p(self.x), dg, self.gwx, ops._p(self.ws), self.ws_bytes)
-        self.wgrad_h.run(ops._p(self.h), dg, self.gwh, ops._p(self.ws), self.ws_bytes)
-        ops.colsum(self.dgates, T * B, 4 * H, 4 * H, self.colsum_scratch, self.gbias)
+        if self.rows_skipped:
+            self.wgrad_x.run_rows(ops._p(self.x), dg, self.gwx, ops._p(self.ws), self.ws_bytes, self.row_prefix, T)
+            self.wgrad_h.run_rows(ops._p(self.h), dg, self.gwh, ops._p(self.ws), self.ws_bytes, self.row_prefix, T)
+            ops.colsum_rows(self.dgates, T, B, 4 * H, 4 * H, self.row_prefix, self.colsum_scratch, self.gbias)
+        else:
+            self.wgrad_x.run(ops._p(self.x), dg, self.gwx, ops._p(self.ws), self.ws_bytes)
+            self.wgrad_h.run(ops._p(self.h), dg, self.gwh, ops._p(self.ws), self.ws_bytes)
+            ops.colsum(self.dgates, T * B, 4 * H, 4 * H, self.colsum_scratch, self.gbias)
         if self.trainable_embedding:
             self.x_dgrad.run(dg, self.wx, ops._p(self.dx))
             ops.embedding_grad(self.dx, self.texts, self.gtable, B, T, self.D, time_major=True)
diff --git a/tumblr_emotions_amd/ops.py b/tumblr_emotions_amd/ops.py
--- a/tumblr_emotions_amd/ops.py
+++ b/tumblr_emotions_amd/ops.py
@@ -497,6 +497,10 @@
         _lib.check(_lib.load().ds_conv_wgrad(C.byref(self.d), x, dz, self.lddz, dw, ws, ws_bytes, _stream()),
                    "ds_conv_wgrad")
 
+    def run_rows(self, x, dz, dw, ws, ws_bytes, row_prefix, T):
+        _lib.check(_lib.load().ds_conv_wgrad_rows(C.byref(self.d), x, dz, self.lddz, dw, ws, ws_bytes, _p(row_prefix), T,
+                                                  _stream()), "ds_conv_wgrad_rows")
+
 
 def bn_finalize(stats, P, count, C_, beta, eps, decay, mean, rstd, shift, mm, mv, pivot=None):
     _lib.check(_lib.load().ds_bn_finalize(_p(stats), P, count, C_, _p(beta), _p(pivot), eps, decay, _p(mean),
@@ -728,7 +732,11 @@
                "ds_lstm_seq_bwd")
 
 
-def seq_sort_desc(seq_len, B, T, perm, len_sorted):
+def seq_sort_desc(seq_len, B, T, perm, len_sorted, row_prefix=None):
+    if row_prefix is not None:
+        _lib.check(_lib.load().ds_seq_sort_desc_rows(_p(seq_len), B, T, _p(perm), _p(len_sorted), _p(row_prefix), _stream()),
+                   "ds_seq_sort_desc_rows")
+        return
     _lib.check(_lib.load().ds_seq_sort_desc(_p(seq_len), B, T, _p(perm), _p(len_sorted), _stream()), "ds_seq_sort_desc")
 
 
@@ -765,6 +773,11 @@
     _lib.check(_lib.load().ds_colsum(_p(x), M, C_, ld, _p(scratch), _p(out), _stream()), "ds_colsum")
 
 
+def colsum_rows(x, T, B, C_, ld, row_prefix, scratch, out):
+    _lib.check(_lib.load().ds_colsum_rows(_p(x), T, B, C_, ld, _p(row_prefix), _p(scratch), _p(out), _stream()),
+               "ds_colsum_rows")
+
+
 def copy2d(src, lds, dst, ldd, rows, cols):
     _lib.check(_lib.load().ds_copy2d(_p(src), lds, _p(dst), ldd, rows, cols, _stream()), "ds_copy2d")
 
```

Result: no change. 19750 samples/s, median of 6 (+0.9%).
